# qope/SIPP

Measured on AMD Instinct MI355X. Metric: SIPP proof-gen wall-clock + pairings-aggregated/sec, n=128 (the 3 STARK sub-proofs, hardened G1/G2 AIRs; outer plonky2 proof not included), higher is better.
Workload: dtype u64; 1 GPU; n=128 SIPP instance per GPU: G1ExpStark 127 IO (N=2^16, W+P+Q=1176), G2ExpStark 127 IO (N=2^16, 2314), Fq12ExpStark 14 IO (N=2^13, 7970); IO records on host -> 3 flat proofs on host, the 3 sub-proofs on 3 concurrent HIP streams; parallelism=1 independent SIPP instance(s), one per GPU, no collective

## Files before the change

### sipp_amd/csrc/api.hip

```cpp
#include <algorithm>
#include <string>

#include "ctx.hpp"
#include "host_poseidon.hpp"

int sipp_poseidon_init_constants(sipp_ctx* ctx);

extern "C" {

void sipp_default_config(sipp_stark_config* cfg) {
    if (!cfg) return;
    cfg->rate_bits = 1;
    cfg->cap_height = 4;
    cfg->pow_bits = 16;
    cfg->arity_bits = 4;
    cfg->final_poly_bits = 5;
    cfg->num_queries = 84;
    cfg->num_challenges = 2;
    cfg->pow_rule = SIPP_POW_DUPLEX;
    cfg->fs_rule = SIPP_FS_STATEMENT;
    cfg->lookup_rule = SIPP_LOOKUP_INDEPENDENT;
}

static hipError_t create_ctx_stream(int device, int level, hipStream_t* out) {
    int lo = 0, hi = 0;
    (void)hipDeviceGetStreamPriorityRange(&lo, &hi);
    static const int dedicated = [] { const char* e = getenv("SIPP_DEDICATED_QUEUES"); return e ? atoi(e) : 1; }();
    if (level <= 0 && dedicated) {
        hipDeviceProp_t prop;
        if (hipGetDeviceProperties(&prop, device) == hipSuccess && prop.multiProcessorCount > 0 && prop.multiProcessorCount <= 1024) {
            uint32_t mask[32];
            const uint32_t words = ((uint32_t)prop.multiProcessorCount + 31) / 32;
            for (uint32_t i = 0; i < words; i++) {
                const uint32_t left = (uint32_t)prop.multiProcessorCount - 32 * i;
                mask[i] = left >= 32 ? 0xffffffffu : (1u << left) - 1;
            }
            if (hipExtStreamCreateWithCUMask(out, words, mask) == hipSuccess) return hipSuccess;
            (void)hipGetLastError();
        }
    }
    return hipStreamCreateWithPriority(out, hipStreamNonBlocking, level > 0 ? hi : level < 0 ? lo : 0);
}

int sipp_ctx_create(sipp_ctx** out, int device, const sipp_stark_config* cfg, size_t workspace_bytes) {
    if (!out) return SIPP_E_BADARG;
    *out = nullptr;
    int ndev = 0;
    if (hipGetDeviceCount(&ndev) != hipSuccess || ndev <= 0 || device < 0 || device >= ndev) return SIPP_E_HIP;
    sipp_ctx* ctx = new sipp_ctx();
    ctx->device = device;
    if (cfg)
        ctx->cfg = *cfg;
    else
        sipp_default_config(&ctx->cfg);
    if (ctx->cfg.rate_bits < 1 || ctx->cfg.rate_bits > 3 || ctx->cfg.num_challenges != 2 || ctx->cfg.arity_bits < 1 ||
        ctx->cfg.arity_bits > 4 || ctx->cfg.cap_height > 8 || ctx->cfg.pow_bits > 32 || ctx->cfg.pow_rule > SIPP_POW_HASH ||
        ctx->cfg.fs_rule > SIPP_FS_UPSTREAM || ctx->cfg.lookup_rule > SIPP_LOOKUP_SHARED || ctx->cfg.num_queries == 0 || ctx->cfg.num_queries > 1024 || ctx->cfg.final_poly_bits > 12) {
        delete ctx;
        return SIPP_E_UNSUPPORTED;
    }
    auto bail = [&](int rc) {
        hipError_t last = hipGetLastError();
        fprintf(stderr, "sipp_ctx_create(device %d, workspace %zu bytes) failed with status %d (last HIP error: %s)\n", device,
                workspace_bytes, rc, hipGetErrorString(last));
        sipp_ctx_destroy(ctx);
        return rc;
    };
    if (hipSetDevice(device) != hipSuccess) return bail(SIPP_E_HIP);
    if (create_ctx_stream(device, 0, &ctx->stream) != hipSuccess) return bail(SIPP_E_HIP);
    if (workspace_bytes == 0) workspace_bytes = (size_t)24 << 30;
    ctx->arena_size = workspace_bytes;
    if (hipMalloc((void**)&ctx->arena, workspace_bytes) != hipSuccess) return bail(SIPP_E_NOMEM);
    if (hipEventCreate(&ctx->t0) != hipSuccess || hipEventCreate(&ctx->t1) != hipSuccess) return bail(SIPP_E_HIP);
    ctx->h_pinned_words = (size_t)1 << 23;
    if (hipHostMalloc((void**)&ctx->h_pinned, ctx->h_pinned_words * 8) != hipSuccess) return bail(SIPP_E_NOMEM);
    int rc = sipp_poseidon_init_constants(ctx);
    if (rc != SIPP_OK) return bail(rc);
    *out = ctx;
    return SIPP_OK;
}

void sipp_ctx_destroy(sipp_ctx* ctx) {
    if (!ctx) return;
    if (ctx->async.started) {
        {
            std::unique_lock<std::mutex> lk(ctx->async.mu);
            ctx->async.cv.wait(lk, [&] { return !ctx->async.has_job || ctx->async.done; });
            ctx->async.quit = true;
        }
        ctx->async.cv.notify_all();
        ctx->async.th.join();
    }
    (void)hipSetDevice(ctx->device);
    if (ctx->stream) (void)hipStreamSynchronize(ctx->stream);
    sipp_witness_graph_release(ctx);
    for (auto& kv : ctx->tables) (void)hipFree(kv.second);
    for (auto e : ctx->ev_pool) (void)hipEventDestroy(e);
    if (ctx->t0) (void)hipEventDestroy(ctx->t0);
    if (ctx->t1) (void)hipEventDestroy(ctx->t1);
    if (ctx->h_pinned) (void)hipHostFree(ctx->h_pinned);
    if (ctx->arena) (void)hipFree(ctx->arena);
    if (ctx->aux_stream) (void)hipStreamDestroy(ctx->aux_stream);
    if (ctx->aux2_stream) (void)hipStreamDestroy(ctx->aux2_stream);
    if (ctx->stream) (void)hipStreamDestroy(ctx->stream);
    delete ctx;
}

uint32_t sipp_abi_version(void) { return SIPP_ABI_VERSION; }

int sipp_ctx_create_checked(sipp_ctx** out, int device, const sipp_stark_config* cfg, size_t cfg_size, uint32_t abi_version,
                            size_t workspace_bytes) {
    if (out) *out = nullptr;
    if (abi_version != SIPP_ABI_VERSION || (cfg && cfg_size != sizeof(sipp_stark_config))) return SIPP_E_BADARG;
    return sipp_ctx_create(out, device, cfg, workspace_bytes);
}

int sipp_ctx_set_kernel_routes(sipp_ctx* ctx, uint32_t routes) {
    if (!ctx || (routes & ~(uint32_t)(SIPP_ROUTE_OPENINGS_UNGROUPED | SIPP_ROUTE_LDE_COLUMN_WIDE | SIPP_ROUTE_WITNESS_NO_GRAPH))) return SIPP_E_BADARG;
    std::unique_lock<std::mutex> lk(ctx->async.mu);
    if (ctx->async.has_job) {
        lk.unlock();
        return sipp_fail(ctx, SIPP_E_BADARG, "set_kernel_routes: a proof is in flight on this ctx");
    }
    ctx->kernel_routes = routes;
    return SIPP_OK;
}

int sipp_ctx_set_hardened(sipp_ctx* ctx, int on) {
    if (!ctx) return SIPP_E_BADARG;
    std::unique_lock<std::mutex> lk(ctx->async.mu);
    if (ctx->async.has_job) {
        lk.unlock();
        return sipp_fail(ctx, SIPP_E_BADARG, "set_hardened: a proof is in flight on this ctx");
    }
    ctx->hardened = on != 0;
    return SIPP_OK;
}

int sipp_ctx_set_stream_priority(sipp_ctx* ctx, int level) {
    if (!ctx) return SIPP_E_BADARG;
    {
        std::unique_lock<std::mutex> lk(ctx->async.mu);
        if (ctx->async.has_job) {
            lk.unlock();
            return sipp_fail(ctx, SIPP_E_BADARG, "set_stream_priority: a proof is in flight on this ctx");
        }
    }
    SIPP_CHECK_HIP(ctx, hipSetDevice(ctx->device));
    hipStream_t ns = nullptr;
    if (create_ctx_stream(ctx->device, level, &ns) != hipSuccess) return sipp_fail(ctx, SIPP_E_HIP, "set_stream_priority: no stream");
    if (ctx->stream) {
        (void)hipStreamSynchronize(ctx->stream);
        if (ctx->prof) {
            (void)sipp_profile_enable(ctx, 0);
            ctx->prof = true;
        }
        (void)hipStreamDestroy(ctx->stream);
    }
    ctx->stream = ns;
    return SIPP_OK;
}

const char* sipp_last_error(const sipp_ctx* ctx) { return ctx ? ctx->err : "null ctx"; }

int sipp_sync(sipp_ctx* ctx) {
    if (!ctx) return SIPP_E_BADARG;
    SIPP_CHECK_HIP(ctx, hipSetDevice(ctx->device));
    SIPP_CHECK_HIP(ctx, hipStreamSynchronize(ctx->stream));
    return SIPP_OK;
}

void* sipp_stream(sipp_ctx* ctx) { return ctx ? (void*)ctx->stream : nullptr; }

static void prof_drain(sipp_ctx* ctx) {
    if (ctx->pending.empty()) return;
    (void)hipSetDevice(ctx->device);
    (void)hipStreamSynchronize(ctx->stream);
    for (auto& p : ctx->pending) {
        float ms = 0.f;
        if (hipEventElapsedTime(&ms, ctx->ev_pool[std::get<1>(p)], ctx->ev_pool[std::get<2>(p)]) == hipSuccess) {
            auto& e = ctx->prof_acc[std::get<0>(p)];
            e.calls++;
// ... 176 lines not shown
```

### sipp_amd/csrc/ctx.hpp

```cpp
#pragma once
#include <stdlib.h>
#include <hip/hip_runtime.h>
#include <stdint.h>
#include <stdio.h>
#include <string.h>

#include <condition_variable>
#include <map>
#include <mutex>
#include <string>
#include <thread>
#include <tuple>
#include <vector>

#include "../../include/sipp_hip.h"
#include "gl.hpp"

struct sipp_gate {
    std::mutex mu;
    std::condition_variable cv;
    bool open = false;
    void release() {
        {
            std::lock_guard<std::mutex> lk(mu);
            open = true;
        }
        cv.notify_all();
    }
    void wait() {
        std::unique_lock<std::mutex> lk(mu);
        cv.wait(lk, [&] { return open; });
    }
};

struct sipp_prof_entry {
    int calls = 0;
    double ms = 0.0;
};

struct sipp_ctx {
    int device = 0;
    hipStream_t stream = nullptr;
    sipp_stark_config cfg{};
    char err[512] = {0};

    char* arena = nullptr;
    size_t arena_size = 0;
    size_t arena_off = 0;
    size_t arena_peak = 0;

    std::map<std::tuple<int, uint64_t, uint64_t>, uint64_t*> tables;

    bool prof = false;
    std::vector<hipEvent_t> ev_pool;
    size_t ev_used = 0;
    std::vector<std::tuple<std::string, size_t, size_t>> pending;
    std::map<std::string, sipp_prof_entry> prof_acc;
    hipEvent_t t0 = nullptr, t1 = nullptr;

    uint64_t* h_pinned = nullptr;
    size_t h_pinned_words = 0;

    sipp_gate* gate_wait = nullptr;
    sipp_gate* gate_release = nullptr;

    hipStream_t aux_stream = nullptr;
    hipStream_t aux2_stream = nullptr;
    struct Fold {
        bool active = false;
        size_t mark = 0;
        uint32_t* d_ios[2] = {nullptr, nullptr};
        void* rows[2] = {nullptr, nullptr};
        int* d_err = nullptr;
        uint32_t num_io[2] = {0, 0};
        size_t n_in[2] = {0, 0};
    } fold;

    bool outputs_only = false;
    bool hardened = false;
    uint32_t kernel_routes = 0;
    struct WitnessGraph {
        hipGraph_t graph = nullptr;
        hipGraphExec_t exec = nullptr;
        std::vector<uint64_t> key;
    } wgraph;

    struct Async {
        std::thread th;
        std::mutex mu;
        std::condition_variable cv;
        bool started = false, has_job = false, done = false, quit = false;
        int kind = 0;
        const uint32_t* ios = nullptr;
        size_t num_io = 0, cap = 0, len = 0;
        uint64_t* out = nullptr;
        int rc = 0;
    } async;
};

#define SIPP_CHECK_HIP(ctx, expr)                                                                   \
    do {                                                                                            \
        hipError_t e__ = (expr);                                                                    \
        if (e__ != hipSuccess) {                                                                    \
            snprintf((ctx)->err, sizeof((ctx)->err), "%s:%d: %s -> %s", __FILE__, __LINE__, #expr,  \
                     hipGetErrorString(e__));                                                       \
            return SIPP_E_HIP;                                                                      \
        }                                                                                           \
    } while (0)

#define SIPP_TRY(expr)              \
    do {                            \
        int rc__ = (expr);          \
        if (rc__ != SIPP_OK) return rc__; \
    } while (0)

static inline int sipp_fail(sipp_ctx* ctx, int code, const char* msg) {
    if (ctx) snprintf(ctx->err, sizeof(ctx->err), "%s", msg);
    return code;
}

struct ArenaMark {
    size_t off;
};
static inline ArenaMark arena_mark(sipp_ctx* ctx) { return ArenaMark{ctx->arena_off}; }
static inline void arena_release(sipp_ctx* ctx, ArenaMark m) { ctx->arena_off = m.off; }
static inline void* arena_alloc(sipp_ctx* ctx, size_t bytes) {
    size_t off = (ctx->arena_off + 255) & ~(size_t)255;
    if (off + bytes > ctx->arena_size) {
        snprintf(ctx->err, sizeof(ctx->err), "workspace arena exhausted: need %zu more bytes (size %zu, used %zu)",
                 bytes, ctx->arena_size, off);
        return nullptr;
    }
    ctx->arena_off = off + bytes;
    if (ctx->arena_off > ctx->arena_peak) ctx->arena_peak = ctx->arena_off;
    return ctx->arena + off;
}
struct ArenaScope {
    sipp_ctx* ctx;
    ArenaMark mark;
    explicit ArenaScope(sipp_ctx* c) : ctx(c), mark(arena_mark(c)) {}
    ~ArenaScope() { arena_release(ctx, mark); }
    ArenaScope(const ArenaScope&) = delete;
    ArenaScope& operator=(const ArenaScope&) = delete;
};
// ... 86 lines not shown
```

### sipp_amd/csrc/fri.hip

```cpp
#include <algorithm>

#include "prover.hpp"

static size_t tree_words(uint32_t log_leaves) { return ((size_t)8 << log_leaves); }

static int read_cap(sipp_ctx* ctx, const uint64_t* d_tree, uint32_t log_leaves, uint32_t cap_height, uint64_t* cap_host) {
    const uint32_t ch = std::min(cap_height, log_leaves);
    uint64_t off = 0;
    for (uint32_t l = 0; l < log_leaves - ch; l++) off += (uint64_t)1 << (log_leaves - l);
    SIPP_CHECK_HIP(ctx, hipMemcpyAsync(cap_host, d_tree + 4 * off, ((size_t)4 << ch) * 8, hipMemcpyDeviceToHost, ctx->stream));
    SIPP_CHECK_HIP(ctx, hipStreamSynchronize(ctx->stream));
    return SIPP_OK;
}

size_t sipp_fri_core_words(const FriParamsDev& p, uint32_t log_n, const uint32_t* leaf_words, int n_oracles) {
    const uint32_t log_m = log_n + p.rate_bits;
    const size_t cap = (size_t)4 << p.cap_height;
    uint32_t sum = 0;
    for (uint32_t ab : p.arity_bits) sum += ab;
    size_t w = p.arity_bits.size() * cap + 2 * ((size_t)1 << (log_n - sum)) + 1;
    size_t per_q = 0;
    for (int o = 0; o < n_oracles; o++) per_q += leaf_words[o] + (size_t)(log_m - p.cap_height) * 4;
    uint32_t lt = log_m;
    for (uint32_t ab : p.arity_bits) {
        lt -= ab;
        per_q += ((size_t)2 << ab) + (size_t)(lt > p.cap_height ? lt - p.cap_height : 0) * 4;
    }
    return w + p.num_queries * per_q;
}

int sipp_fri_prove_core(sipp_ctx* ctx, const FriOracleDev* ors, int n_oracles, uint32_t log_n, const FriParamsDev& p,
                        uint64_t* d_final, host::Challenger& ch, uint64_t* pf, size_t& pos, size_t cap_total, size_t* final_len,
                        const std::function<void(const char*)>& tick) {
    const uint32_t log_m = log_n + p.rate_bits, R = (uint32_t)p.arity_bits.size(), nq = p.num_queries;
    const size_t n = (size_t)1 << log_n, m = (size_t)1 << log_m;
    const size_t cap_words = (size_t)4 << p.cap_height;
    if (p.cap_height > 8 || n_oracles < 1 || n_oracles > 8) return sipp_fail(ctx, SIPP_E_UNSUPPORTED, "fri: unsupported shape");
    auto push = [&](const uint64_t* v, size_t cnt) -> int {
        if (pos + cnt > cap_total) return SIPP_E_BUFSZ;
        memcpy(pf + pos, v, cnt * 8);
        pos += cnt;
        return SIPP_OK;
    };
    uint64_t cap_host[4 << 8];
    std::vector<uint64_t*> r_vals(R), r_tree(R);
    std::vector<uint32_t> r_loglen(R);
    uint64_t* cur = d_final;
    size_t len_c = n;
    uint32_t log_len = log_m;
    uint64_t shift = gl::GEN;
    for (uint32_t r = 0; r < R; r++) {
        const uint32_t ab = p.arity_bits[r];
        const size_t len = (size_t)1 << log_len;
        if (log_len < ab + 0u || (len_c >> ab) == 0) return sipp_fail(ctx, SIPP_E_BADARG, "fri: reduction arities exceed the degree");
        r_loglen[r] = log_len;
        r_vals[r] = arena_alloc_t<uint64_t>(ctx, 2 * len);
        r_tree[r] = arena_alloc_t<uint64_t>(ctx, tree_words(log_len - ab));
        uint64_t* nxt = arena_alloc_t<uint64_t>(ctx, 2 * (len_c >> ab) + 2);
        if (!r_vals[r] || !r_tree[r] || !nxt) return SIPP_E_NOMEM;
        SIPP_TRY(sipp_ntt_dif(ctx, cur, len_c, log_len - p.rate_bits, r_vals[r], len, log_len, 2, false, NttDiag{shift, 0}));
        SIPP_TRY(sipp_k_fri_leaves(ctx, r_vals[r], len, ab, r_tree[r]));
        SIPP_TRY(sipp_k_merkle_levels(ctx, r_tree[r], log_len - ab, p.cap_height));
        SIPP_TRY(read_cap(ctx, r_tree[r], log_len - ab, p.cap_height, cap_host));
        const size_t cw = (size_t)4 << std::min(p.cap_height, log_len - ab);
        ch.observe_many(cap_host, cw);
        SIPP_TRY(push(cap_host, cw));
        const gl::E2 fb = ch.get_ext();
        SIPP_TRY(sipp_k_fri_fold(ctx, cur, len_c, ab, fb, nxt));
        cur = nxt;
        len_c >>= ab;
        log_len -= ab;
        shift = gl::pow(shift, (uint64_t)1 << ab);
    }
    (void)cap_words;
    if (final_len) *final_len = len_c;
    {
        std::vector<uint64_t> fpv(2 * len_c);
        SIPP_CHECK_HIP(ctx, hipMemcpyAsync(fpv.data(), cur, fpv.size() * 8, hipMemcpyDeviceToHost, ctx->stream));
        SIPP_CHECK_HIP(ctx, hipStreamSynchronize(ctx->stream));
        for (size_t i = 0; i < len_c; i++) {
            uint64_t e[2] = {fpv[i], fpv[len_c + i]};
            ch.observe_many(e, 2);
            SIPP_TRY(push(e, 2));
        }
    }
    if (tick) tick("fri commit phase");
    uint64_t pow_witness = 0;
    if (p.pow_rule == SIPP_POW_HASH) {
        uint64_t zero[12] = {0}, cur_h[4];
        for (int i = 0; i < 4; i++) cur_h[i] = ch.get();
        SIPP_TRY(sipp_k_pow_search(ctx, zero, cur_h, 4, 0, p.pow_bits, &pow_witness));
    } else {
        SIPP_TRY(sipp_k_pow_search(ctx, ch.state, ch.in_buf, ch.n_in, 7, p.pow_bits, &pow_witness));
        ch.observe(pow_witness);
        (void)ch.get();
    }
    SIPP_TRY(push(&pow_witness, 1));
    if (tick) tick("pow");
    std::vector<uint32_t> qidx(nq);
    for (uint32_t i = 0; i < nq; i++) qidx[i] = (uint32_t)(ch.get() % m);
    uint32_t* d_idx = arena_alloc_t<uint32_t>(ctx, nq);
    if (!d_idx) return SIPP_E_NOMEM;
    SIPP_CHECK_HIP(ctx, hipMemcpyAsync(d_idx, qidx.data(), nq * 4, hipMemcpyHostToDevice, ctx->stream));
    const uint32_t nsib0 = log_m - p.cap_height;
    size_t st_words = 0;
    std::vector<size_t> off_rows(n_oracles), off_sib(n_oracles), off_leaf(R), off_rsib(R);
    std::vector<uint32_t> rsib(R), rshift(R);
    for (int o = 0; o < n_oracles; o++) {
        off_rows[o] = st_words;
        st_words += (size_t)nq * ors[o].ncols;
        off_sib[o] = st_words;
        st_words += (size_t)nq * nsib0 * 4;
    }
    {
        uint32_t sh = 0;
        for (uint32_t r = 0; r < R; r++) {
            const uint32_t ab = p.arity_bits[r];
            sh += ab;
            rshift[r] = sh;
            const uint32_t lt = log_m - sh;
            rsib[r] = lt > p.cap_height ? lt - p.cap_height : 0;
            off_leaf[r] = st_words;
            st_words += (size_t)nq * ((size_t)2 << ab);
            off_rsib[r] = st_words;
            st_words += (size_t)nq * rsib[r] * 4;
        }
    }
    if (st_words > ctx->h_pinned_words) return sipp_fail(ctx, SIPP_E_NOMEM, "query staging exceeds the pinned buffer");
    uint64_t* d_st = arena_alloc_t<uint64_t>(ctx, st_words);
    if (!d_st) return SIPP_E_NOMEM;
    std::vector<QueryGatherTask> tasks;
    {
        for (int o = 0; o < n_oracles; o++) {
            tasks.push_back(QueryGatherTask{ors[o].lde, d_st + off_rows[o], (uint64_t)ors[o].stride, 0, ors[o].ncols, 0, 0});
            if (nsib0) tasks.push_back(QueryGatherTask{ors[o].tree, d_st + off_sib[o], 0, 1, log_m, nsib0, 0});
        }
        for (uint32_t r = 0; r < R; r++) {
            const uint32_t ab = p.arity_bits[r];
            tasks.push_back(QueryGatherTask{r_vals[r], d_st + off_leaf[r], (uint64_t)1 << r_loglen[r], 2, rshift[r], ab, 0});
            if (rsib[r]) tasks.push_back(QueryGatherTask{r_tree[r], d_st + off_rsib[r], 0, 1, r_loglen[r] - ab, rsib[r], rshift[r]});
        }
        QueryGatherTask* d_tasks = arena_alloc_t<QueryGatherTask>(ctx, tasks.size());
        if (!d_tasks) return SIPP_E_NOMEM;
        SIPP_CHECK_HIP(ctx, hipMemcpyAsync(d_tasks, tasks.data(), tasks.size() * sizeof(QueryGatherTask), hipMemcpyHostToDevice, ctx->stream));
        SIPP_TRY(sipp_k_gather_tasks(ctx, d_tasks, (uint32_t)tasks.size(), d_idx, nq));
    }
    uint64_t* hst = ctx->h_pinned;
    SIPP_CHECK_HIP(ctx, hipMemcpyAsync(hst, d_st, st_words * 8, hipMemcpyDeviceToHost, ctx->stream));
    SIPP_CHECK_HIP(ctx, hipStreamSynchronize(ctx->stream));
    for (uint32_t qi = 0; qi < nq; qi++) {
        for (int o = 0; o < n_oracles; o++) {
            SIPP_TRY(push(hst + off_rows[o] + (size_t)qi * ors[o].ncols, (size_t)ors[o].ncols));
            SIPP_TRY(push(hst + off_sib[o] + (size_t)qi * nsib0 * 4, (size_t)nsib0 * 4));
        }
        for (uint32_t r = 0; r < R; r++) {
            const size_t lw = (size_t)2 << p.arity_bits[r];
            SIPP_TRY(push(hst + off_leaf[r] + (size_t)qi * lw, lw));
            SIPP_TRY(push(hst + off_rsib[r] + (size_t)qi * rsib[r] * 4, (size_t)rsib[r] * 4));
        }
    }
    return SIPP_OK;
}


#define SIPP_FRI_MAGIC 0x5349505046524931ULL

static size_t batch_len(const sipp_fri_batch& b) {
    size_t k = 0;
    for (uint32_t r = 0; r < b.n_ranges; r++) k += b.ranges[r].col_end - b.ranges[r].col_begin;
    return k;
}

static int check_params(sipp_ctx* ctx, const sipp_fri_params* p, uint32_t log_n) {
    if (!p || p->rate_bits < 1 || p->rate_bits > 3 || p->cap_height > 8 || p->pow_bits > 32 || p->pow_rule > SIPP_POW_HASH ||
        p->num_queries == 0 || p->num_queries > 1024 || p->n_rounds > SIPP_FRI_MAX_ROUNDS)
        return sipp_fail(ctx, SIPP_E_UNSUPPORTED, "fri: parameters out of the supported range");
    uint32_t sum = 0;
    for (uint32_t r = 0; r < p->n_rounds; r++) {
        if (p->arity_bits[r] < 1 || p->arity_bits[r] > 4) return sipp_fail(ctx, SIPP_E_UNSUPPORTED, "fri: arity must be 2, 4, 8 or 16");
        sum += p->arity_bits[r];
        if (log_n + p->rate_bits < sum + p->cap_height)
            return sipp_fail(ctx, SIPP_E_BADARG, "fri: reduction arities leave a layer smaller than its cap");
        if (log_n + p->rate_bits - sum + p->arity_bits[r] < 4)
            return sipp_fail(ctx, SIPP_E_UNSUPPORTED, "fri: a committed layer of fewer than 16 values is not supported");
    }
    if (sum > log_n) return sipp_fail(ctx, SIPP_E_BADARG, "fri: the reduction arities exceed the degree bits");
    if (log_n < 10 || log_n > 24) return sipp_fail(ctx, SIPP_E_UNSUPPORTED, "fri: degree bits outside the supported range [10, 24]");
    return SIPP_OK;
}

extern "C" {

void sipp_fri_const_arity(sipp_fri_params* p, uint32_t arity_bits, uint32_t final_poly_bits, uint32_t degree_bits) {
    if (!p) return;
    p->n_rounds = 0;
    while (degree_bits > final_poly_bits && degree_bits + p->rate_bits - arity_bits >= p->cap_height && degree_bits >= arity_bits &&
           p->n_rounds < SIPP_FRI_MAX_ROUNDS) {
        p->arity_bits[p->n_rounds++] = arity_bits;
        degree_bits -= arity_bits;
    }
}

int sipp_commit_batch_ex(sipp_ctx* ctx, const uint64_t* d_in, int from_coeffs, uint64_t* d_coeffs, uint64_t* d_lde, uint64_t* d_tree,
                         size_t ncols, uint32_t log_n, uint32_t rate_bits, uint32_t cap_height, const uint64_t* d_salt,
                         uint32_t n_salt, uint64_t* cap_out) {
    if (!ctx || !d_in || !d_coeffs || !d_lde || !d_tree || !cap_out || ncols == 0) return SIPP_E_BADARG;
    if (rate_bits < 1 || rate_bits > 3 || cap_height > 8 || (n_salt != 0 && (n_salt != SIPP_SALT_SIZE || !d_salt)))
        return sipp_fail(ctx, SIPP_E_UNSUPPORTED, "commit_batch_ex: blowup 2 / 4 / 8, cap height <= 8, salt 0 or 4 columns");
    SIPP_CHECK_HIP(ctx, hipSetDevice(ctx->device));
    const uint32_t log_m = log_n + rate_bits;
    const size_t n = (size_t)1 << log_n, m = (size_t)1 << log_m;
    ArenaScope scope(ctx);
    int rc;
    if (from_coeffs) {
        if (d_in != d_coeffs) SIPP_CHECK_HIP(ctx, hipMemcpyAsync(d_coeffs, d_in, ncols * n * 8, hipMemcpyDeviceToDevice, ctx->stream));
        rc = sipp_lde_from_coeffs(ctx, d_coeffs, d_lde, ncols, log_n, rate_bits);
        if (rc == SIPP_E_UNSUPPORTED) rc = sipp_ntt_dif(ctx, d_coeffs, n, log_n, d_lde, m, log_m, ncols, false, NttDiag{gl::GEN, 0});
    } else {
        rc = d_in != d_coeffs ? sipp_lde_from_values(ctx, d_in, d_coeffs, d_lde, ncols, log_n, rate_bits) : SIPP_E_UNSUPPORTED;
        if (rc == SIPP_E_UNSUPPORTED) {
            const uint64_t* src = d_in;
            if (d_in == d_coeffs) {
                uint64_t* tmp = arena_alloc_t<uint64_t>(ctx, n * ncols);
                if (!tmp) return SIPP_E_NOMEM;
                SIPP_CHECK_HIP(ctx, hipMemcpyAsync(tmp, d_in, n * ncols * 8, hipMemcpyDeviceToDevice, ctx->stream));
                src = tmp;
            }
            rc = sipp_bitrev_cols(ctx, src, n, d_coeffs, n, log_n, ncols);
            if (rc == SIPP_OK) rc = sipp_ntt_dit(ctx, d_coeffs, n, log_n, ncols, true, NttDiag{});
// ... 12 lines not shown
                           uint32_t log_n, const sipp_fri_params* p) {
    if (!oracles || !batches || !p || n_oracles == 0 || n_oracles > 8 || n_batches == 0) return 0;
    FriParamsDev fp;
    fp.rate_bits = p->rate_bits; fp.cap_height = p->cap_height; fp.pow_bits = p->pow_bits; fp.num_queries = p->num_queries;
    fp.pow_rule = p->pow_rule;
    uint32_t sum = 0;
    for (uint32_t r = 0; r < p->n_rounds && r < SIPP_FRI_MAX_ROUNDS; r++) {
        fp.arity_bits.push_back(p->arity_bits[r]);
        sum += p->arity_bits[r];
    }
    if (sum > log_n) return 0;
    uint32_t lw[8];
    for (size_t o = 0; o < n_oracles; o++) lw[o] = oracles[o].n_polys + oracles[o].n_salt;
    size_t w = 8 + sipp_fri_core_words(fp, log_n, lw, (int)n_oracles);
    for (size_t b = 0; b < n_batches; b++) w += 2 * batch_len(batches[b]);
    return w;
}

int sipp_fri_prove_openings(sipp_ctx* ctx, const sipp_oracle* oracles, size_t n_oracles, const sipp_fri_batch* batches,
                            size_t n_batches, uint32_t log_n, const sipp_fri_params* p, sipp_challenger* chs, uint64_t* proof_out,
                            size_t proof_cap, size_t* proof_len) {
    if (!ctx || !oracles || !batches || !p || !chs || !proof_out || !proof_len || n_oracles == 0 || n_oracles > 8 || n_batches == 0)
        return SIPP_E_BADARG;
    SIPP_CHECK_HIP(ctx, hipSetDevice(ctx->device));
    SIPP_TRY(check_params(ctx, p, log_n));
    if (chs->n_in > 7 || chs->n_out > 8) return sipp_fail(ctx, SIPP_E_BADARG, "fri: malformed challenger state");
    const size_t total = sipp_fri_proof_size(oracles, n_oracles, batches, n_batches, log_n, p);
    if (total == 0) return SIPP_E_BADARG;
    if (proof_cap < total) return sipp_fail(ctx, SIPP_E_BUFSZ, "fri: proof buffer too small (see sipp_fri_proof_size)");
    for (size_t b = 0; b < n_batches; b++)
        for (uint32_t r = 0; r < batches[b].n_ranges; r++) {
            const sipp_poly_range& rg = batches[b].ranges[r];
            if (rg.oracle >= n_oracles || rg.col_begin > rg.col_end || rg.col_end > oracles[rg.oracle].n_polys)
                return sipp_fail(ctx, SIPP_E_BADARG, "fri: polynomial range outside its oracle");
        }
    const size_t n = (size_t)1 << log_n, m = n << p->rate_bits;
    FriParamsDev fp;
    fp.rate_bits = p->rate_bits; fp.cap_height = p->cap_height; fp.pow_bits = p->pow_bits; fp.num_queries = p->num_queries;
    fp.pow_rule = p->pow_rule;
    for (uint32_t r = 0; r < p->n_rounds; r++) fp.arity_bits.push_back(p->arity_bits[r]);
    host::Challenger ch;
    memcpy(ch.state, chs->state, sizeof ch.state);
    memcpy(ch.in_buf, chs->in_buf, sizeof ch.in_buf);
    memcpy(ch.out_buf, chs->out_buf, sizeof ch.out_buf);
    ch.n_in = (uint32_t)chs->n_in;
    ch.n_out = (uint32_t)chs->n_out;
    struct Release {
        sipp_ctx* c;
        ArenaMark mk;
        ~Release() {
            (void)hipStreamSynchronize(c->stream);
            arena_release(c, mk);
        }
    } release{ctx, arena_mark(ctx)};
    size_t pos = 0;
    uint64_t* pf = proof_out;
    {
        uint64_t hdr[8] = {SIPP_FRI_MAGIC, p->n_rounds, 0, p->num_queries, (uint64_t)n_oracles, (uint64_t)n_batches, total, log_n};
        memcpy(pf, hdr, sizeof hdr);
        pos = 8;
    }
    std::vector<uint64_t*> d_zp(n_batches), d_zip(n_batches);
    std::vector<gl::E2> points(n_batches);
    for (size_t b = 0; b < n_batches; b++) {
        points[b] = gl::E2{batches[b].point[0], batches[b].point[1]};
        if (gl::eq(gl::pow(points[b], (uint64_t)n), gl::e2(1))) return sipp_fail(ctx, SIPP_E_SUBGROUP, "fri: opening point in the subgroup");
        d_zp[b] = arena_alloc_t<uint64_t>(ctx, 2 * n);
        d_zip[b] = arena_alloc_t<uint64_t>(ctx, 2 * n);
        if (!d_zp[b] || !d_zip[b]) return SIPP_E_NOMEM;
        SIPP_TRY(sipp_k_pow_table(ctx, points[b], n, d_zp[b]));
        SIPP_TRY(sipp_k_pow_table(ctx, gl::inv(points[b]), n, d_zip[b]));
    }
    for (size_t b = 0; b < n_batches; b++) {
        const size_t k = batch_len(batches[b]);
        uint64_t* d_open = arena_alloc_t<uint64_t>(ctx, 4 * k + 4);
        if (!d_open) return SIPP_E_NOMEM;
        size_t at = 0;
        for (uint32_t r = 0; r < batches[b].n_ranges; r++) {
            const sipp_poly_range& rg = batches[b].ranges[r];
            const size_t cnt = rg.col_end - rg.col_begin;
            SIPP_TRY(sipp_k_openings(ctx, oracles[rg.oracle].d_coeffs + (size_t)rg.col_begin * n, cnt, n, d_zp[b], nullptr, d_open + 4 * at));
            at += cnt;
        }
        std::vector<uint64_t> hop(4 * k + 4);
        SIPP_CHECK_HIP(ctx, hipMemcpyAsync(hop.data(), d_open, (4 * k) * 8, hipMemcpyDeviceToHost, ctx->stream));
        SIPP_CHECK_HIP(ctx, hipStreamSynchronize(ctx->stream));
        for (size_t j = 0; j < k; j++) {
            memcpy(pf + pos, &hop[4 * j], 16);
            pos += 2;
            ch.observe_many(&hop[4 * j], 2);
        }
    }
    const gl::E2 alpha = ch.get_ext();
    uint64_t* d_acc = arena_alloc_t<uint64_t>(ctx, 2 * n);
    uint64_t* d_final = arena_alloc_t<uint64_t>(ctx, 2 * n);
    if (!d_acc || !d_final) return SIPP_E_NOMEM;
    for (size_t b = 0; b < n_batches; b++) {
        const size_t k = batch_len(batches[b]);
        std::vector<const uint64_t*> cols;
        cols.reserve(k);
        for (uint32_t r = 0; r < batches[b].n_ranges; r++) {
            const sipp_poly_range& rg = batches[b].ranges[r];
            for (uint32_t c = rg.col_begin; c < rg.col_end; c++) cols.push_back(oracles[rg.oracle].d_coeffs + (size_t)c * n);
        }
        std::vector<uint32_t> apow(6 * k + 6);
        gl::E2 ap = gl::e2(1);
        for (size_t c = 0; c < k; c++) {
            const uint64_t comp[2] = {ap.c0, ap.c1};
            for (int q = 0; q < 2; q++) {
                apow[6 * c + 3 * q] = (uint32_t)comp[q] & 0x3FFFFFu;
                apow[6 * c + 3 * q + 1] = (uint32_t)(comp[q] >> 22) & 0x3FFFFFu;
                apow[6 * c + 3 * q + 2] = (uint32_t)(comp[q] >> 44);
            }
            ap = gl::mul(ap, alpha);
        }
        const uint64_t** d_cols = reinterpret_cast<const uint64_t**>(arena_alloc(ctx, (k + 1) * sizeof(uint64_t*)));
        uint32_t* d_apow = arena_alloc_t<uint32_t>(ctx, apow.size());
        if (!d_cols || !d_apow) return SIPP_E_NOMEM;
        SIPP_CHECK_HIP(ctx, hipMemcpyAsync(d_cols, cols.data(), k * sizeof(uint64_t*), hipMemcpyHostToDevice, ctx->stream));
        SIPP_CHECK_HIP(ctx, hipMemcpyAsync(d_apow, apow.data(), apow.size() * 4, hipMemcpyHostToDevice, ctx->stream));
        SIPP_CHECK_HIP(ctx, hipStreamSynchronize(ctx->stream));
        SIPP_TRY(sipp_k_fri_batch_quotient(ctx, d_cols, (int)k, n, d_apow, d_zp[b], d_zip[b], ap, b == 0, d_acc));
    }
    SIPP_TRY(sipp_k_fri_mulx(ctx, d_acc, n, d_final));
    FriOracleDev ors[8];
    for (size_t o = 0; o < n_oracles; o++)
        ors[o] = FriOracleDev{oracles[o].d_lde, m, oracles[o].n_polys + oracles[o].n_salt, oracles[o].d_tree};
    size_t flen = 0;
    SIPP_TRY(sipp_fri_prove_core(ctx, ors, (int)n_oracles, log_n, fp, d_final, ch, pf, pos, total, &flen, nullptr));
    pf[2] = flen;
    if (pos != total) return sipp_fail(ctx, SIPP_E_BUFSZ, "internal: opening proof length mismatch");
    *proof_len = pos;
    memcpy(chs->state, ch.state, sizeof ch.state);
    memcpy(chs->in_buf, ch.in_buf, sizeof ch.in_buf);
    memcpy(chs->out_buf, ch.out_buf, sizeof ch.out_buf);
    chs->n_in = ch.n_in;
    chs->n_out = ch.n_out;
    return SIPP_OK;
}

}
```

### sipp_amd/csrc/poseidon.hip

```cpp
#include <type_traits>
#include "ctx.hpp"
#ifndef GLL_T
#define GLL_T 140
#endif
#include "poseidon.hpp"
#include "poseidon_pair.hpp"
#include "prover.hpp"

namespace {

#ifndef SIPP_LEAVES_WPE
#define SIPP_LEAVES_WPE 3
#endif
__global__ void __launch_bounds__(256) __attribute__((amdgpu_waves_per_eu(SIPP_LEAVES_WPE, SIPP_LEAVES_WPE)))
poseidon_leaves_kernel(const uint64_t* __restrict__ lde, size_t col_stride,
                                                             uint32_t ncols, uint64_t n_leaves,
                                                             uint64_t* __restrict__ digests) {
    const uint64_t j0 = (uint64_t)blockIdx.x * blockDim.x + threadIdx.x;
    const uint64_t j = j0 < n_leaves ? j0 : n_leaves - 1;
    uint64_t s[12];
#pragma unroll
    for (int i = 0; i < 12; i++) s[i] = 0;
    const uint64_t* p = lde + j;
    __shared__ uint64_t stash[11 * 256];
// ... 190 lines not shown
    const uint32_t words = 2u << ab;
    const uint64_t* c0 = vals + (k << ab);
    const uint64_t* c1 = vals + len + (k << ab);
    uint64_t s[12];
#pragma unroll
    for (int i = 0; i < 12; i++) s[i] = 0;
    if (words <= 4) {
        s[0] = c0[0];
        s[1] = c1[0];
        if (words == 4) {
            s[2] = c0[1];
            s[3] = c1[1];
        }
    } else {
#pragma unroll 1
        for (uint32_t chunk = 0; chunk < words / 8; chunk++) {
#pragma unroll
            for (int e = 0; e < 8; e++) s[e] = (e & 1) ? c1[4 * chunk + (e >> 1)] : c0[4 * chunk + (e >> 1)];
            poseidon::permute(s);
        }
    }
    uint64_t* d = digests + 4 * k;
    d[0] = s[0]; d[1] = s[1]; d[2] = s[2]; d[3] = s[3];
}

struct PowArgs {
    uint64_t state[12];
    uint64_t in_buf[8];
    uint32_t n_in, pow_bits, resp_word;
    uint64_t base;
    unsigned long long* result;
};
__global__ void __launch_bounds__(256) pow_kernel(PowArgs a) {
    const uint64_t w = a.base + (uint64_t)blockIdx.x * blockDim.x + threadIdx.x;
    uint64_t s[12];
#pragma unroll
    for (int i = 0; i < 12; i++) s[i] = a.state[i];
#pragma unroll
    for (int i = 0; i < 8; i++) {
        if ((uint32_t)i < a.n_in) s[i] = a.in_buf[i];
        if ((uint32_t)i == a.n_in) s[i] = w;
    }
    poseidon::permute(s);
    const uint64_t resp = a.resp_word == 7 ? s[7] : s[0];
    if ((resp >> (64 - a.pow_bits)) == 0) atomicMin(a.result, (unsigned long long)w);
}

constexpr uint64_t thin_threshold() { return 65536; }

}

int sipp_k_fri_leaves(sipp_ctx* ctx, const uint64_t* d_vals, size_t len, uint32_t arity_bits, uint64_t* d_digests) {
    uint64_t nl = len >> arity_bits;
    ProfScope ps(ctx, "fri_leaves");
    if (arity_bits != 4) {
        if (arity_bits < 1 || arity_bits > 4) return sipp_fail(ctx, SIPP_E_UNSUPPORTED, "fri_leaves: arity must be 2, 4, 8 or 16");
        hipLaunchKernelGGL(fri_leaves_any_kernel, dim3((unsigned)((nl + 63) / 64)), dim3(64), 0, ctx->stream, d_vals, (uint64_t)len,
                           arity_bits, d_digests);
    } else if (nl <= thin_threshold())
        hipLaunchKernelGGL(fri_leaves_pair_kernel, dim3((unsigned)((2 * nl + 255) / 256)), dim3(256), 0, ctx->stream, d_vals,
                           (uint64_t)len, d_digests);
    else
        hipLaunchKernelGGL(fri_leaves_kernel, dim3((unsigned)((nl + 63) / 64)), dim3(64), 0, ctx->stream, d_vals, (uint64_t)len,
                           d_digests);
    SIPP_CHECK_HIP(ctx, hipGetLastError());
    return SIPP_OK;
}

int sipp_k_pow_search(sipp_ctx* ctx, const uint64_t state[12], const uint64_t* in_buf, uint32_t n_in, uint32_t resp_word,
                      uint32_t pow_bits, uint64_t* witness) {
    if (pow_bits == 0) { *witness = 0; return SIPP_OK; }
    if (pow_bits > 32 || n_in > 7 || (resp_word != 0 && resp_word != 7))
        return sipp_fail(ctx, SIPP_E_UNSUPPORTED, "pow_search: unsupported parameters");
    ArenaMark mk = arena_mark(ctx);
    unsigned long long* d_res = arena_alloc_t<unsigned long long>(ctx, 1);
    if (!d_res) return SIPP_E_NOMEM;
    PowArgs a;
    memcpy(a.state, state, sizeof a.state);
    memset(a.in_buf, 0, sizeof a.in_buf);
    memcpy(a.in_buf, in_buf, n_in * sizeof(uint64_t));
    a.n_in = n_in; a.pow_bits = pow_bits; a.resp_word = resp_word; a.result = d_res;
    const uint32_t log_batch = pow_bits + 1 < 12 ? 12 : pow_bits + 1 > 28 ? 28 : pow_bits + 1;
    const uint64_t batch = (uint64_t)1 << log_batch;
    unsigned long long h_res = ~0ull;
    SIPP_CHECK_HIP(ctx, hipMemsetAsync(d_res, 0xff, sizeof(unsigned long long), ctx->stream));
    for (uint64_t base = 0; base < ((uint64_t)1 << 44); base += batch) {
        a.base = base;
        {
            ProfScope ps(ctx, "pow_grind");
            hipLaunchKernelGGL(pow_kernel, dim3((unsigned)(batch / 256)), dim3(256), 0, ctx->stream, a);
        }
        SIPP_CHECK_HIP(ctx, hipGetLastError());
        SIPP_CHECK_HIP(ctx, hipMemcpyAsync(&h_res, d_res, sizeof h_res, hipMemcpyDeviceToHost, ctx->stream));
        SIPP_CHECK_HIP(ctx, hipStreamSynchronize(ctx->stream));
        if (h_res != ~0ull) break;
    }
    arena_release(ctx, mk);
    if (h_res == ~0ull) return sipp_fail(ctx, SIPP_E_UNSUPPORTED, "pow_search: no witness found");
    *witness = (uint64_t)h_res;
    return SIPP_OK;
}

int sipp_poseidon_init_constants(sipp_ctx* ctx) {
    SIPP_CHECK_HIP(ctx, hipMemcpyToSymbol(HIP_SYMBOL(poseidon::c_rc), SIPP_POSEIDON_RC, sizeof(SIPP_POSEIDON_RC)));
    SIPP_CHECK_HIP(ctx, hipMemcpyToSymbol(HIP_SYMBOL(poseidon::c_fast_first), SIPP_POSEIDON_FAST_FIRST,
                                          sizeof(SIPP_POSEIDON_FAST_FIRST)));
    SIPP_CHECK_HIP(ctx, hipMemcpyToSymbol(HIP_SYMBOL(poseidon::c_fast_scalar), SIPP_POSEIDON_FAST_SCALAR,
                                          sizeof(SIPP_POSEIDON_FAST_SCALAR)));
    SIPP_CHECK_HIP(ctx, hipMemcpyToSymbol(HIP_SYMBOL(poseidon::c_fast_mi), SIPP_POSEIDON_FAST_MI,
                                          sizeof(SIPP_POSEIDON_FAST_MI)));
    SIPP_CHECK_HIP(ctx, hipMemcpyToSymbol(HIP_SYMBOL(poseidon::c_fast_vs), SIPP_POSEIDON_FAST_VS,
                                          sizeof(SIPP_POSEIDON_FAST_VS)));
    SIPP_CHECK_HIP(ctx, hipMemcpyToSymbol(HIP_SYMBOL(poseidon::c_fast_what), SIPP_POSEIDON_FAST_WHAT,
                                          sizeof(SIPP_POSEIDON_FAST_WHAT)));
    SIPP_CHECK_HIP(ctx, hipMemcpyToSymbol(HIP_SYMBOL(poseidon::c_blk3), SIPP_POSEIDON_BLK3, sizeof(SIPP_POSEIDON_BLK3)));
    SIPP_CHECK_HIP(ctx, hipMemcpyToSymbol(HIP_SYMBOL(poseidon::c_comb3), SIPP_POSEIDON_COMB3, sizeof(SIPP_POSEIDON_COMB3)));
    SIPP_CHECK_HIP(ctx, hipMemcpyToSymbol(HIP_SYMBOL(poseidon::c_comb_c), SIPP_POSEIDON_COMB_C, sizeof(SIPP_POSEIDON_COMB_C)));
    SIPP_CHECK_HIP(ctx, hipMemcpyToSymbol(HIP_SYMBOL(poseidon::d_dense_a), SIPP_POSEIDON_DENSE_A, sizeof(SIPP_POSEIDON_DENSE_A)));
    SIPP_CHECK_HIP(ctx, hipMemcpyToSymbol(HIP_SYMBOL(poseidon::c_dense_start), SIPP_POSEIDON_DENSE_START, sizeof(SIPP_POSEIDON_DENSE_START)));
    SIPP_CHECK_HIP(ctx, hipMemcpyToSymbol(HIP_SYMBOL(poseidon_pair::d_pair_a), SIPP_POSEIDON_PAIR_A, sizeof(SIPP_POSEIDON_PAIR_A)));
    SIPP_CHECK_HIP(ctx, hipMemcpyToSymbol(HIP_SYMBOL(poseidon_pair::d_pair_mds_a), SIPP_POSEIDON_PAIR_MDS_A, sizeof(SIPP_POSEIDON_PAIR_MDS_A)));
    SIPP_CHECK_HIP(ctx, hipMemcpyToSymbol(HIP_SYMBOL(poseidon_pair::d_pair_cc), SIPP_POSEIDON_PAIR_CC3, sizeof(SIPP_POSEIDON_PAIR_CC3)));
    SIPP_CHECK_HIP(ctx, hipMemcpyToSymbol(HIP_SYMBOL(poseidon_pair::d_pair_start), SIPP_POSEIDON_PAIR_START, sizeof(SIPP_POSEIDON_PAIR_START)));
    return SIPP_OK;
}

int sipp_k_poseidon_leaves(sipp_ctx* ctx, const uint64_t* d_lde, size_t col_stride, size_t ncols, uint32_t log_leaves,
                           uint64_t* d_digests) {
    if (ncols == 0 || ncols > 0xffffffffull) return sipp_fail(ctx, SIPP_E_BADARG, "poseidon_leaves: bad ncols");
    uint64_t n = (uint64_t)1 << log_leaves;
    const bool thin = ncols > 4 && n <= thin_threshold() && n >= 32;
    ProfScope ps(ctx, ncols <= 4 ? "poseidon_leaves_noop" : thin ? "poseidon_leaves_pair" : "poseidon_leaves");
    if (ncols <= 4) {
        hipLaunchKernelGGL(poseidon_leaves_copy_kernel, dim3((unsigned)((n + 255) / 256)), dim3(256), 0, ctx->stream, d_lde, col_stride,
                           (uint32_t)ncols, n, d_digests);
    } else if (thin) {
        unsigned grid = (unsigned)((2 * n + 255) / 256);
        hipLaunchKernelGGL(poseidon_leaves_pair_kernel, dim3(grid), dim3(256), 0, ctx->stream, d_lde, col_stride,
                           (uint32_t)ncols, n, d_digests);
    } else {
        const unsigned bs = n <= 65536 ? 64 : 256;
        unsigned grid = (unsigned)((n + bs - 1) / bs);
        hipLaunchKernelGGL(poseidon_leaves_kernel, dim3(grid), dim3(bs), 0, ctx->stream, d_lde, col_stride,
                           (uint32_t)ncols, n, d_digests);
    }
    SIPP_CHECK_HIP(ctx, hipGetLastError());
    return SIPP_OK;
}

int sipp_k_merkle_levels(sipp_ctx* ctx, uint64_t* d_tree, uint32_t log_leaves, uint32_t cap_height) {
    if (cap_height > log_leaves) cap_height = log_leaves;
    {
        uint32_t level = 0;
        const uint32_t top = log_leaves - cap_height;
        while (level < top) {
            const uint32_t log_nodes = log_leaves - level;
            uint32_t lw = log_nodes <= 10 ? log_nodes : log_nodes >= 18 ? 10 : 8;
            uint32_t nlev = lw < top - level ? lw : top - level;
            const uint64_t widest_parents = (uint64_t)1 << (log_nodes - 1);
            if (widest_parents > thin_threshold()) {
                lw = 11;
                nlev = 3 < top - level ? 3 : top - level;
            }
            const unsigned blocks = 1u << (log_nodes - lw);
            ProfScope ps(ctx, "merkle_subtree");
            if (widest_parents <= thin_threshold())
                hipLaunchKernelGGL(merkle_subtree_kernel<true>, dim3(blocks), dim3(256), 0, ctx->stream, d_tree, log_leaves, level, lw, nlev);
            else
                hipLaunchKernelGGL(merkle_subtree_kernel<false>, dim3(blocks), dim3(256), 0, ctx->stream, d_tree, log_leaves, level, lw, nlev);
            SIPP_CHECK_HIP(ctx, hipGetLastError());
            level += nlev;
        }
        return SIPP_OK;
    }
}

// ... 9 lines not shown
```

### sipp_amd/csrc/prover.hip

```cpp
#include <map>

#include "ctx.hpp"
#include "prover.hpp"

namespace {

using gl::E2;

template <bool REV>
__device__ __forceinline__ uint64_t block_scan_mul_256(uint64_t v, uint64_t* s) {
    const int t = REV ? 255 - (int)threadIdx.x : (int)threadIdx.x;
    s[t] = v;
    __syncthreads();
    for (int off = 1; off < 256; off <<= 1) {
        uint64_t o = t >= off ? s[t - off] : 1;
        __syncthreads();
        v = gl::mul(v, o);
        s[t] = v;
        __syncthreads();
    }
    return v;
}

__device__ __forceinline__ void block_scan4_mul_256(uint64_t (&v)[4], uint64_t (*s)[256]) {
// ... 299 lines not shown
            const uint64_t coef = gl::from_i64(*w++);
            uint64_t va[16], vb[16];
            w += qvec<16>(w, c, va);
            w += qvec<16>(w, c, vb);
#pragma unroll
            for (int ch = 0; ch < 2; ch++) {
                gl::Acc6 Ae, Ao, Be, Bo;
                Ae.zero(); Ao.zero(); Be.zero(); Bo.zero();
#pragma unroll
                for (int i = 0; i < 8; i++) {
                    const uint32_t* g3 = a.ginv3[ch][i];
                    Ae.mac((uint32_t)va[2 * i], (uint32_t)(va[2 * i] >> 32), g3);
                    Ao.mac((uint32_t)va[2 * i + 1], (uint32_t)(va[2 * i + 1] >> 32), g3);
                    Be.mac((uint32_t)vb[2 * i], (uint32_t)(vb[2 * i] >> 32), g3);
                    Bo.mac((uint32_t)vb[2 * i + 1], (uint32_t)(vb[2 * i + 1] >> 32), g3);
                }
                const uint64_t ae = Ae.reduce(), ao = Ao.reduce(), be = Be.reduce(), bo = Bo.reduce();
                const uint64_t cross = gl::add(gl::mul(ae, bo), gl::mul(ao, be));
                uint64_t t = gl::mad(gl::mul(ao, bo), a.gamma_inv[ch], gl::mul(ae, be));
                t = gl::mad(cross, 65536, t);
                psum[ch] = gl::mad(coef, t, psum[ch]);
            }
        }
        const int nl = slice == 0 ? (int)*w++ : 0;
        for (int p = 0; p < nl; p++) {
            const uint64_t coef = gl::from_i64(*w++);
            uint64_t va[16];
            w += qvec<16>(w, c, va);
#pragma unroll
            for (int ii = 0; ii < 16; ii++) e[ii] = gl::mad(coef, va[ii], e[ii]);
        }
        if (slice == 0) {
        uint64_t q[17];
        (void)qvec<17>(qdesc, c, q);
        const uint64_t s = c.local(sign_col);
        const uint64_t sgn = gl::sub(1, gl::add(s, s));
        uint64_t cprev = 0;
        const uint64_t coff = gl::from_i64(coffset);
        uint64_t d[32];
#pragma unroll
        for (int k = 0; k < 32; k++) {
            uint64_t al = 0, ah = 0;
#pragma unroll
            for (int ii = 0; ii < 17; ii++) {
                const int jj = k - ii;
                if (jj >= 0 && jj < 16) {
                    al += (uint64_t)(uint32_t)q[ii] * a.p_limbs[jj];
                    ah += (uint64_t)(uint32_t)(q[ii] >> 32) * a.p_limbs[jj];
                }
            }
            const uint64_t l = al + (ah << 32);
            const uint32_t h = (uint32_t)(ah >> 32) + (l < al ? 1u : 0u);
            const uint64_t qp = gl::reduce96(h, l);
            d[k] = gl::sub(e[k], gl::mul(sgn, qp));
        }
        const uint64_t wgt = (uint64_t)1 << (16 * grp);
#pragma unroll
        for (int mm = 0; mm < 32; mm++) {
            if (mm < 32 / grp) {
                uint64_t v;
                if (grp == 2) v = gl::mad(d[(2 * mm + 1) & 31], 65536, d[(2 * mm) & 31]);
                else v = d[mm];
                uint64_t ck = 0;
                if (mm < 32 / grp - 1) {
                    for (int l = 0; l < ncl; l++)
                        ck = gl::mad(c.local(cbase + mm * ncl + l), (uint64_t)1 << (lb * l), ck);
                    ck = gl::sub(ck, coff);
                }
                v = gl::sub(v, cprev);
                v = gl::mad(ck, wgt, v);
                c.emit(v);
                cprev = ck;
            }
        }
        c.emit(gl::mul(s, gl::sub(s, 1)));
        }
        c.acc0 = gl::mad(a.alpha16[0], psum[0], c.acc0);
        c.acc1 = gl::mad(a.alpha16[1], psum[1], c.acc1);
    }
    a.part[((size_t)g * 2 + 0) * m + j] = gl::mul(c.acc0, a.seg_pow[2 * g]);
    a.part[((size_t)g * 2 + 1) * m + j] = gl::mul(c.acc1, a.seg_pow[2 * g + 1]);
}

__global__ void alpha_pow3_kernel(uint64_t a0, uint64_t a1, int K, int nc, uint32_t* __restrict__ out) {
    const int t = blockIdx.x * blockDim.x + threadIdx.x;
    const int total = 2 * 3 + nc * 2 * 6;
    if (t >= total) return;
    int c, e;
    if (t < 6) {
        c = t / 3;
        e = K - 1 - t % 3;
    } else {
        const int k = (t - 6) / 12, r = (t - 6) % 12, slot = r % 6;
        c = r / 6;
        e = K - 1 - (3 + 2 * k) - (slot >> 1) * 2 * nc - (slot & 1);
    }
    uint32_t l[3];
    gl::limbs3(l, gl::pow(c ? a1 : a0, (uint64_t)e));
    for (int q = 0; q < 3; q++) out[3 * t + q] = l[q];
}

struct RestAcc {
    gl::Acc6 a[2];
    int terms;
    uint64_t folded[2];
    __device__ __forceinline__ void init() {
        a[0].zero();
        a[1].zero();
        terms = 0;
        folded[0] = folded[1] = 0;
    }
    __device__ __forceinline__ void mac(uint64_t v, const uint32_t* __restrict__ p0, const uint32_t* __restrict__ p1) {
        const uint32_t lo = (uint32_t)v, hi = (uint32_t)(v >> 32);
        a[0].mac(lo, hi, p0);
        a[1].mac(lo, hi, p1);
    }
    __device__ __forceinline__ void maybe_fold(int added) {
        terms += added;
        if (terms >= 960) {
            for (int c = 0; c < 2; c++) {
                folded[c] = gl::add(folded[c], gl::canon(a[c].reduce()));
                a[c].zero();
            }
            terms = 0;
        }
    }
    __device__ __forceinline__ uint64_t value(int c) const { return gl::add(folded[c], gl::canon(a[c].reduce())); }
};

struct RestPoint {
    uint64_t lf, zl, ll, zh_inv;
};
__device__ __forceinline__ RestPoint rest_point(const QuotArgs& a, uint32_t i) {
    const uint64_t x = gl::mul(gl::GEN, gl::pow(a.w_m, i));
    const uint64_t zh = a.zh[i & 1];
    RestPoint r;
    r.zl = gl::sub(x, a.g_inv);
    r.lf = gl::mul(gl::mul(zh, a.ninv), gl::inv(gl::sub(x, 1)));
    r.ll = gl::mul(gl::mul(gl::mul(zh, a.ninv), a.g_inv), gl::inv(r.zl));
    r.zh_inv = a.zh_inv[i & 1];
    return r;
}
__device__ __forceinline__ void rest_store(const QuotArgs& a, size_t m, size_t j, const RestPoint& pt, const uint64_t F[2], const uint64_t T[2],
                                           const uint64_t R[2]) {
    uint64_t acc[2] = {0, 0};
    for (int g = 0; g < a.n_seg; g++) {
        acc[0] = gl::add(acc[0], a.part[((size_t)g * 2 + 0) * m + j]);
        acc[1] = gl::add(acc[1], a.part[((size_t)g * 2 + 1) * m + j]);
    }
#pragma unroll
    for (int q = 0; q < 2; q++) {
        uint64_t v = gl::mul(acc[q], a.alphaK[q]);
        v = gl::add(v, R[q]);
        v = gl::mad(pt.lf, F[q], v);
        v = gl::mad(pt.zl, T[q], v);
        a.out[(size_t)q * m + j] = gl::mul(v, pt.zh_inv);
    }
}

template <bool SPLIT>
__global__ void __launch_bounds__(256) quotient_rest_kernel(QuotArgs a) {
    const size_t m = (size_t)1 << a.log_m;
    constexpr uint32_t RB = 3, RW = 256u >> RB;
    const uint32_t tid = threadIdx.x, run = tid / RW, blk = blockIdx.x, half = blk / (uint32_t)(m >> 9);
    const size_t j = (size_t)half * (m >> 1) + (size_t)run * (m >> (RB + 1)) + (size_t)(blk % (uint32_t)(m >> 9)) * RW + tid % RW;
    const uint32_t i = gl::bitrev((uint32_t)j, a.log_m);
    QCtx c;
    c.lde = a.lde;
    c.lde_stride = a.lde_stride;
    c.alpha0 = a.alpha[0];
// ... 192 lines not shown
    } else {
        col = a.coeffs[2] + (size_t)(b - a.ncols[0] - a.ncols[1]) * a.n;
        t1 = nullptr;
    }
    openings_column(col, a.n, a.t0, t1, a.n, a.out + (size_t)b * 4);
}

constexpr int OG = 4;
struct OpenGArgs {
    const uint64_t* coeffs[3];
    uint32_t ncols[3];
    size_t n, seg_len;
    const uint64_t *t0, *t1;
    uint64_t* partial;
};
__global__ void __launch_bounds__(256) openings_group_kernel(OpenGArgs a) {
    __shared__ uint64_t s[4][256];
    uint32_t g = blockIdx.x, orc = 0, col_base = 0;
    while (orc < 2 && g >= (a.ncols[orc] + OG - 1) / OG) {
        g -= (a.ncols[orc] + OG - 1) / OG;
        col_base += a.ncols[orc];
        orc++;
    }
    const uint32_t c0 = g * OG, cnt = min((uint32_t)OG, a.ncols[orc] - c0);
    const bool two = orc < 2;
    const size_t n = a.n, lo = (size_t)blockIdx.y * a.seg_len, hi = min(n, lo + a.seg_len);
    const uint64_t* col = a.coeffs[orc] + (size_t)c0 * n;
    gl::Acc160 acc[OG][4];
    constexpr int OB = 2;
    size_t k = lo + threadIdx.x;
    for (; k + (OB - 1) * 256 < hi; k += OB * 256) {
        uint64_t p0[OB], p1[OB], q0[OB], q1[OB], v[OB][OG];
#pragma unroll
        for (int b = 0; b < OB; b++) {
            const size_t kb = k + (size_t)b * 256;
            p0[b] = a.t0[kb];
            p1[b] = a.t0[n + kb];
            q0[b] = two ? a.t1[kb] : 0;
            q1[b] = two ? a.t1[n + kb] : 0;
#pragma unroll
            for (int c = 0; c < OG; c++) v[b][c] = (uint32_t)c < cnt ? col[(size_t)c * n + kb] : 0;
        }
#pragma unroll
        for (int b = 0; b < OB; b++)
#pragma unroll
            for (int c = 0; c < OG; c++) {
                if ((uint32_t)c >= cnt) break;
                acc[c][0].mac(v[b][c], p0[b]);
                acc[c][1].mac(v[b][c], p1[b]);
                if (two) {
                    acc[c][2].mac(v[b][c], q0[b]);
                    acc[c][3].mac(v[b][c], q1[b]);
                }
            }
    }
    for (; k < hi; k += 256) {
        const uint64_t p0 = a.t0[k], p1 = a.t0[n + k], q0 = two ? a.t1[k] : 0, q1 = two ? a.t1[n + k] : 0;
#pragma unroll
        for (int c = 0; c < OG; c++) {
            if ((uint32_t)c >= cnt) break;
            const uint64_t v = col[(size_t)c * n + k];
            acc[c][0].mac(v, p0);
            acc[c][1].mac(v, p1);
            if (two) {
                acc[c][2].mac(v, q0);
                acc[c][3].mac(v, q1);
            }
        }
    }
#pragma unroll
    for (int c = 0; c < OG; c++) {
        if ((uint32_t)c >= cnt) break;
#pragma unroll
        for (int q = 0; q < 4; q++) s[q][threadIdx.x] = gl::canon(acc[c][q].reduce());
        __syncthreads();
        for (int off = 128; off > 0; off >>= 1) {
            if ((int)threadIdx.x < off)
                for (int q = 0; q < 4; q++) s[q][threadIdx.x] = gl::add(s[q][threadIdx.x], s[q][threadIdx.x + off]);
            __syncthreads();
        }
        if (threadIdx.x < 4) a.partial[((size_t)(col_base + c0 + c) * gridDim.y + blockIdx.y) * 4 + threadIdx.x] = s[threadIdx.x][0];
        __syncthreads();
    }
}

struct CombArgs {
    const uint64_t* src[3];
    int cnt[3];
    size_t n;
    const uint32_t* apow3;
    int n1;
    int slices;
    uint64_t* partial;
};
__global__ void __launch_bounds__(256) fri_combine_kernel(CombArgs a) {
    const size_t k = (size_t)blockIdx.x * 256 + threadIdx.x;
    const int total = a.cnt[0] + a.cnt[1] + a.cnt[2];
    const int per = (total + a.slices - 1) / a.slices;
    const int c_lo = blockIdx.y * per, c_hi = min(total, c_lo + per);
    gl::Acc6 G0, G1, H0, H1;
    G0.zero(); G1.zero(); H0.zero(); H1.zero();
    const uint64_t *src0 = a.src[0], *src1 = a.src[1], *src2 = a.src[2];
    const int cnt0 = a.cnt[0], cnt01 = a.cnt[0] + a.cnt[1], n1 = a.n1;
    const size_t nn = a.n;
    const uint32_t* __restrict__ apow3 = a.apow3;
    auto col_of = [=](int c) -> const uint64_t* {
        return c < cnt0 ? src0 + (size_t)c * nn : c < cnt01 ? src1 + (size_t)(c - cnt0) * nn : src2 + (size_t)(c - cnt01) * nn;
    };
#define SIPP_COMB_TERM(cc, vv)                                             \
    do {                                                                   \
        const uint64_t v_ = (vv);                                          \
        const uint32_t lo_ = (uint32_t)v_, hi_ = (uint32_t)(v_ >> 32);     \
        const uint32_t* __restrict__ w_ = apow3 + 6 * (cc);                \
        if ((cc) < n1) {                                 \
            G0.mac(lo_, hi_, w_);                                          \
            G1.mac(lo_, hi_, w_ + 3);                                      \
        } else {                                                           \
            H0.mac(lo_, hi_, w_);                                          \
            H1.mac(lo_, hi_, w_ + 3);                                      \
        }                                                                  \
    } while (0)
    constexpr int CB = 8;
    int c = c_lo;
    for (; c + CB <= c_hi; c += CB) {
        uint64_t v[CB];
#pragma unroll
        for (int b = 0; b < CB; b++) v[b] = col_of(c + b)[k];
#pragma unroll
        for (int b = 0; b < CB; b++) SIPP_COMB_TERM(c + b, v[b]);
    }
    for (; c < c_hi; c++) SIPP_COMB_TERM(c, col_of(c)[k]);
#undef SIPP_COMB_TERM
    const uint64_t g0 = gl::canon(G0.reduce()), g1 = gl::canon(G1.reduce());
    uint64_t* p = a.partial + (size_t)blockIdx.y * 4 * a.n;
    p[k] = gl::add(g0, gl::canon(H0.reduce()));
    p[a.n + k] = gl::add(g1, gl::canon(H1.reduce()));
    p[2 * a.n + k] = g0;
    p[3 * a.n + k] = g1;
}

struct GCombArgs {
    const uint64_t* const* cols;
    int total;
    size_t n;
    const uint32_t* apow3;
    int slices;
    uint64_t* partial;
};
__global__ void __launch_bounds__(256) fri_gcombine_kernel(GCombArgs a) {
    const size_t k = (size_t)blockIdx.x * 256 + threadIdx.x;
    const int per = (a.total + a.slices - 1) / a.slices;
    const int c_lo = blockIdx.y * per, c_hi = min(a.total, c_lo + per);
    gl::Acc6 G0, G1;
    G0.zero(); G1.zero();
    for (int c = c_lo; c < c_hi; c++) {
        const uint64_t v = a.cols[c][k];
        const uint32_t lo = (uint32_t)v, hi = (uint32_t)(v >> 32);
        const uint32_t* __restrict__ w = a.apow3 + 6 * c;
        G0.mac(lo, hi, w);
        G1.mac(lo, hi, w + 3);
    }
    uint64_t* p = a.partial + (size_t)blockIdx.y * 4 * a.n;
    p[k] = gl::canon(G0.reduce());
    p[a.n + k] = gl::canon(G1.reduce());
}

// ... 167 lines not shown
            const uint32_t l = e >> 2, w = e & 3;
            size_t off = 0;
            for (uint32_t k = 0; k < l; k++) off += (size_t)1 << (t.b - k);
            const size_t node = ((x >> t.d) >> l) ^ 1;
            t.out[((size_t)q * t.c + l) * 4 + w] = t.src[(off + node) * 4 + w];
        }
    } else {
        const size_t leaf = x >> t.b;
        for (uint32_t e = threadIdx.x; e < (2u << t.c); e += blockDim.x)
            t.out[((size_t)q << (t.c + 1)) + e] = t.src[(size_t)(e & 1) * t.a + (leaf << t.c) + (e >> 1)];
    }
}

}

int sipp_k_gather_tasks(sipp_ctx* ctx, const QueryGatherTask* d_tasks, uint32_t n_tasks, const uint32_t* d_idx, uint32_t nq) {
    if (!n_tasks || !nq) return SIPP_OK;
    ProfScope ps(ctx, "query_gather");
    hipLaunchKernelGGL(gather_tasks_kernel, dim3(nq, n_tasks), dim3(256), 0, ctx->stream, d_tasks, d_idx);
    SIPP_CHECK_HIP(ctx, hipGetLastError());
    return SIPP_OK;
}

int sipp_k_z_columns(sipp_ctx* ctx, const air_spec_t* a, const uint64_t* d_trace, uint32_t log_n, const uint64_t beta[2],
                     const uint64_t gamma[2], uint64_t* d_zv) {
    const size_t n = (size_t)1 << log_n;
    const int P = 2 * a->n_checked;
    const int zr = (n >= 16384) ? 8 : 4;
    const size_t zblock = (size_t)256 * zr;
    const unsigned nblk = (unsigned)(n / zblock);
    if (n % zblock) return sipp_fail(ctx, SIPP_E_BADARG, "z_columns: n must be a multiple of 1024");
    ArenaScope scope(ctx);
    uint64_t* totals = arena_alloc_t<uint64_t>(ctx, (size_t)2 * P * nblk);
    if (!totals) return SIPP_E_NOMEM;
    {
        ProfScope ps(ctx, "z_phase_a");
        if (zr == 8)
            hipLaunchKernelGGL(z_phase_a<8>, dim3(nblk, P / 2), dim3(256), 0, ctx->stream, d_trace, n, a->n_main, a->n_checked,
                               a->checked_base, gamma[0], gamma[1], beta[0], beta[1], d_zv, totals);
        else
            hipLaunchKernelGGL(z_phase_a<4>, dim3(nblk, P / 2), dim3(256), 0, ctx->stream, d_trace, n, a->n_main, a->n_checked,
                               a->checked_base, gamma[0], gamma[1], beta[0], beta[1], d_zv, totals);
    }
    {
        ProfScope ps(ctx, "z_phase_bc");
        hipLaunchKernelGGL(z_phase_b, dim3(P), dim3(256), 0, ctx->stream, totals, (int)nblk);
        if (zr == 8)
            hipLaunchKernelGGL(z_phase_c<8>, dim3(nblk, P), dim3(256), 0, ctx->stream, d_zv, n, totals);
        else
            hipLaunchKernelGGL(z_phase_c<4>, dim3(nblk, P), dim3(256), 0, ctx->stream, d_zv, n, totals);
    }
    SIPP_CHECK_HIP(ctx, hipGetLastError());
    return SIPP_OK;
}

static void host_ntt(uint64_t* a, uint32_t log_n, bool inverse) {
    const size_t n = (size_t)1 << log_n;
    for (size_t i = 0; i < n; i++) {
        const size_t j = gl::bitrev((uint32_t)i, log_n);
        if (i < j) std::swap(a[i], a[j]);
    }
    uint64_t root = gl::root_of_unity(log_n);
    if (inverse) root = gl::inv(root);
    for (uint32_t s = 1; s <= log_n; s++) {
        const size_t mlen = (size_t)1 << s, h = mlen >> 1;
        uint64_t wm = root;
        for (uint32_t k = s; k < log_n; k++) wm = gl::sqr(wm);
        for (size_t k = 0; k < n; k += mlen) {
            uint64_t w = 1;
            for (size_t j = 0; j < h; j++) {
                const uint64_t t = gl::mul(w, a[k + j + h]), u = a[k + j];
                a[k + j] = gl::add(u, t);
                a[k + j + h] = gl::sub(u, t);
                w = gl::mul(w, wm);
            }
        }
    }
    if (inverse) {
        const uint64_t ninv = gl::inv((uint64_t)n);
        for (size_t i = 0; i < n; i++) a[i] = gl::mul(a[i], ninv);
    }
}

int sipp_k_quotient(sipp_ctx* ctx, const air_spec_t* a, uint32_t log_n, const uint64_t* d_lde, const uint64_t* d_zlde,
                    size_t lde_stride, const uint64_t* d_aux, const uint64_t alpha[2], const uint64_t beta[2],
                    const uint64_t gamma[2], uint64_t* d_out) {
    const uint32_t log_m = log_n + 1;
    const size_t n = (size_t)1 << log_n, m = (size_t)1 << log_m;
    QuotArgs q{};
    q.lde = d_lde; q.zlde = d_zlde; q.aux = d_aux; q.lde_stride = lde_stride;
    q.prog = sipp_air_prog_device(ctx, a);
    if (!q.prog) return SIPP_E_HIP;
    q.prog_len = a->prog_len;
    q.W = a->n_main + 2 * a->n_checked; q.nm = a->n_main; q.nc = a->n_checked; q.cbase = a->checked_base;
    q.tbits = a->table_bits; q.log_n = log_n; q.log_m = log_m;
    q.alpha[0] = alpha[0]; q.alpha[1] = alpha[1]; q.gamma[0] = gamma[0]; q.gamma[1] = gamma[1];
    q.beta[0] = beta[0]; q.beta[1] = beta[1];
    const uint64_t g = gl::root_of_unity(log_n), wm = gl::root_of_unity(log_m);
    for (int k = 0; k < AIR_N_PERIODIC; k++) {
        const uint64_t mk = (uint64_t)AIR_PERIODIC[k][0], r0 = (uint64_t)AIR_PERIODIC[k][1];
        uint64_t* t = sipp_table_get(ctx, 200 + k, log_n, 0);
        if (!t) {
            const uint64_t K = n / mk;
            std::vector<uint64_t> v(2 * mk);
            const uint64_t gs = gl::inv(gl::pow(g, r0)), scale = gl::mul(K % gl::P, gl::inv(n % gl::P));
            for (uint64_t i = 0; i < 2 * mk; i++) {
                uint64_t x = gl::mul(gl::GEN, gl::pow(wm, i));
                uint64_t y = gl::mul(x, gs);
                uint64_t num = gl::sub(gl::pow(y, n), 1), den = gl::sub(gl::pow(y, K), 1);
                v[i] = gl::mul(gl::mul(num, gl::inv(den)), scale);
            }
            SIPP_TRY(sipp_table_put(ctx, 200 + k, log_n, 0, v, &t));
        }
        q.per_tab[k] = t;
        q.per_mask[k] = (uint32_t)(2 * mk - 1);
    }
    q.vper_tab = nullptr;
    q.vper_mask = 0;
    if (a->n_vflag + a->n_vconst > 0) {
        const uint32_t lr = (uint32_t)a->log_rows;
        const size_t R = (size_t)1 << lr, R2 = 2 * R;
        const int nv = a->n_vflag + a->n_vconst;
        uint64_t* t = sipp_table_get(ctx, 104, log_n, (uint64_t)a->kind);
        if (!t) {
            std::vector<uint64_t> tab((size_t)nv * R2), col(R2);
            const uint64_t shift = gl::pow(gl::GEN, (uint64_t)1 << (log_n - lr));
            std::map<std::vector<int64_t>, int> seen;
            std::vector<int64_t> vals(R);
            for (int k = 0; k < nv; k++) {
                for (size_t r = 0; r < R; r++) vals[r] = air_vper_value(a, k, (int)r);
                auto it = seen.find(vals);
                if (it != seen.end()) {
                    memcpy(&tab[(size_t)k * R2], &tab[(size_t)it->second * R2], R2 * 8);
                    continue;
                }
                seen.emplace(vals, k);
                for (size_t r = 0; r < R; r++) col[r] = gl::from_i64(vals[r]);
                host_ntt(col.data(), lr, true);
                uint64_t f = 1;
                for (size_t j = 0; j < R; j++) {
                    col[j] = gl::mul(col[j], f);
                    f = gl::mul(f, shift);
                }
                for (size_t j = R; j < R2; j++) col[j] = 0;
                host_ntt(col.data(), lr + 1, false);
                memcpy(&tab[(size_t)k * R2], col.data(), R2 * 8);
            }
            SIPP_TRY(sipp_table_put(ctx, 104, log_n, (uint64_t)a->kind, tab, &t));
        }
        q.vper_tab = t;
        q.vper_mask = (uint32_t)(R2 - 1);
    }
    const uint64_t sN = gl::pow(gl::GEN, n);
    q.zh[0] = gl::sub(sN, 1);
    q.zh[1] = gl::sub(gl::neg(sN), 1);
    q.zh_inv[0] = gl::inv(q.zh[0]);
    q.zh_inv[1] = gl::inv(q.zh[1]);
    q.ninv = gl::inv(n % gl::P);
    q.g_inv = gl::inv(g);
    q.w_m = wm;
    for (int i = 0; i < 16; i++) q.p_limbs[i] = AIR_BN_P_LIMBS[i];
    q.out = d_out;
    for (int ch = 0; ch < 2; ch++) {
        if (alpha[ch] == 0) return sipp_fail(ctx, SIPP_E_UNSUPPORTED, "quotient: a zero constraint challenge");
        const uint64_t gi = gl::inv(alpha[ch]);
        q.gamma_inv[ch] = gi;
        q.alpha16[ch] = gl::pow(alpha[ch], 16);
        uint64_t x = 1;
        for (int i = 0; i < 8; i++) {
            q.ginv3[ch][i][0] = (uint32_t)x & 0x3FFFFFu;
            q.ginv3[ch][i][1] = (uint32_t)(x >> 22) & 0x3FFFFFu;
            q.ginv3[ch][i][2] = (uint32_t)(x >> 44);
            x = gl::mul(x, gi);
        }
    }
    int n_gadget_segs = 0;
    ArenaScope scope(ctx);
    {
        std::vector<uint32_t> off, cnt;
        std::vector<int> ncons;
        const int64_t* w = a->prog;
        const int64_t* end = a->prog + a->prog_len;
        while (w < end && w[0] == 1) {
            off.push_back((uint32_t)(w - a->prog));
            cnt.push_back(0);
            if (w[6] != 2) return sipp_fail(ctx, SIPP_E_UNSUPPORTED, "quotient: gadgets must pair their limbs (group 2)");
            ncons.push_back(32 / (int)w[6] + 1);
            w += 7;
            w += 2 + 5 * w[1];
            int64_t np = *w++;
            for (int64_t p = 0; p < np; p++) {
                w += 1;
                w += 2 + 5 * w[1];
                w += 2 + 5 * w[1];
            }
            int64_t nl = *w++;
            for (int64_t p = 0; p < nl; p++) {
                w += 1;
                w += 2 + 5 * w[1];
            }
            if (np > 64) {
                const uint32_t nsl = (uint32_t)std::min<int64_t>(SIPP_QUOTIENT_MAX_SLICES, (np + 39) / 40);
                cnt.back() = 0x80000000u | (nsl << 8);
                for (uint32_t k = 1; k < nsl; k++) {
                    off.push_back(off.back());
                    cnt.push_back(0x80000000u | (nsl << 8) | k);
                    ncons.push_back(0);
                }
            }
        }
        while (w < end) {
            off.push_back((uint32_t)(w - a->prog));
            uint32_t k = 0;
            while (w < end && k < 64) {
                int64_t nmono = w[1];
                w += 2;
                for (int64_t mo = 0; mo < nmono; mo++) w += 2 + 2 * w[1];
                k++;
            }
            cnt.push_back(k);
            ncons.push_back((int)k);
        }
        const int ns = (int)off.size();
        q.n_seg = ns;
        n_gadget_segs = 0;
        auto is_gadget = [](uint32_t c) { return c == 0 || (c >> 31) != 0; };
        while (n_gadget_segs < ns && is_gadget(cnt[n_gadget_segs])) n_gadget_segs++;
        for (int g = n_gadget_segs; g < ns; g++)
            if (is_gadget(cnt[g])) return sipp_fail(ctx, SIPP_E_UNSUPPORTED, "quotient: gadgets must precede the polynomial constraints");
        std::vector<uint64_t> host((size_t)ns * 2 + ns + 2 + 192, 0);
        int after = 0;
        for (int g = ns - 1; g >= 0; g--) {
            host[2 * g] = gl::pow(alpha[0], (uint64_t)after);
            host[2 * g + 1] = gl::pow(alpha[1], (uint64_t)after);
            after += ncons[g];
        }
        uint32_t* h32 = reinterpret_cast<uint32_t*>(&host[2 * ns]);
        memcpy(h32, off.data(), (size_t)ns * 4);
        memcpy(h32 + ns, cnt.data(), (size_t)ns * 4);
        const size_t ap_at = (size_t)ns * 2 + (((size_t)2 * ns + 1) >> 1);
        {
            uint32_t* ap = reinterpret_cast<uint32_t*>(&host[ap_at]);
            for (int ch = 0; ch < 2; ch++) {
                uint64_t x = 1;
                for (int e = 0; e < 64; e++) {
                    ap[(ch * 64 + e) * 3 + 0] = (uint32_t)x & 0x3FFFFFu;
                    ap[(ch * 64 + e) * 3 + 1] = (uint32_t)(x >> 22) & 0x3FFFFFu;
                    ap[(ch * 64 + e) * 3 + 2] = (uint32_t)(x >> 44);
                    x = gl::mul(x, alpha[ch]);
                }
            }
        }
        uint64_t* d_tab = arena_alloc_t<uint64_t>(ctx, host.size());
        q.part = arena_alloc_t<uint64_t>(ctx, (size_t)ns * 2 * m);
        if (!d_tab || !q.part) return SIPP_E_NOMEM;
        SIPP_CHECK_HIP(ctx, hipMemcpyAsync(d_tab, host.data(), host.size() * 8, hipMemcpyHostToDevice, ctx->stream));
        SIPP_CHECK_HIP(ctx, hipStreamSynchronize(ctx->stream));
        q.seg_pow = d_tab;
        q.seg_off = reinterpret_cast<const uint32_t*>(d_tab + 2 * ns);
        q.seg_cnt = q.seg_off + ns;
        q.apoly3 = reinterpret_cast<const uint32_t*>(d_tab + ap_at);
    }
    {
        q.K = 3 + 6 * a->n_checked;
        const int nw = 6 + 12 * a->n_checked;
        uint32_t* d_ap = arena_alloc_t<uint32_t>(ctx, (size_t)3 * nw);
        if (!d_ap) return SIPP_E_NOMEM;
        hipLaunchKernelGGL(alpha_pow3_kernel, dim3((unsigned)((nw + 255) / 256)), dim3(256), 0, ctx->stream, alpha[0], alpha[1],
                           q.K, a->n_checked, d_ap);
        q.apow3 = d_ap;
        q.alphaK[0] = gl::pow(alpha[0], (uint64_t)q.K);
        q.alphaK[1] = gl::pow(alpha[1], (uint64_t)q.K);
    }
    {
        ProfScope ps(ctx, "quotient_prog");
        if (n_gadget_segs)
            hipLaunchKernelGGL(quotient_prog_kernel<false>, dim3((unsigned)(m / 64), (unsigned)n_gadget_segs), dim3(64), 0, ctx->stream, q, 0);
        if (q.n_seg > n_gadget_segs)
            hipLaunchKernelGGL(quotient_prog_kernel<true>, dim3((unsigned)(m / 64), (unsigned)(q.n_seg - n_gadget_segs)), dim3(64), 0, ctx->stream,
                               q, n_gadget_segs);
    }
    {
        ProfScope ps(ctx, "quotient_rest");
        q.chunks = (int)sipp_quotient_rest_chunks(log_n, a->n_checked);
        if (q.chunks > 1) {
            q.rest_part = arena_alloc_t<uint64_t>(ctx, (size_t)q.chunks * 6 * m);
            if (!q.rest_part) return SIPP_E_NOMEM;
            hipLaunchKernelGGL(quotient_rest_kernel<true>, dim3((unsigned)(m / 256), (unsigned)q.chunks), dim3(256), 0, ctx->stream, q);
            hipLaunchKernelGGL(quotient_finish_kernel, dim3((unsigned)(m / 256)), dim3(256), 0, ctx->stream, q);
        } else {
            q.chunks = 1;
            hipLaunchKernelGGL(quotient_rest_kernel<false>, dim3((unsigned)(m / 256)), dim3(256), 0, ctx->stream, q);
        }
    }
    SIPP_CHECK_HIP(ctx, hipGetLastError());
    return SIPP_OK;
}

int sipp_k_pow_table(sipp_ctx* ctx, gl::E2 base, size_t n, uint64_t* d_tab) {
    ProfScope ps(ctx, "pow_table");
    hipLaunchKernelGGL(pow_table_kernel, dim3((unsigned)((n + 255) / 256)), dim3(256), 0, ctx->stream, base, n, d_tab);
    SIPP_CHECK_HIP(ctx, hipGetLastError());
    return SIPP_OK;
}

int sipp_k_pow_table4(sipp_ctx* ctx, const gl::E2 base[4], size_t n, uint64_t* const d_tab[4]) {
    ProfScope ps(ctx, "pow_table");
    Pow4Args a;
    for (int i = 0; i < 4; i++) {
        a.base[i] = base[i];
        a.tab[i] = d_tab[i];
    }
    a.n = n;
    hipLaunchKernelGGL(pow_table4_kernel, dim3((unsigned)((n + 255) / 256), 4), dim3(256), 0, ctx->stream, a);
    SIPP_CHECK_HIP(ctx, hipGetLastError());
    return SIPP_OK;
}

int sipp_k_openings(sipp_ctx* ctx, const uint64_t* d_coeffs, size_t ncols, size_t n, const uint64_t* d_t0,
                    const uint64_t* d_t1, uint64_t* d_out) {
    if (!ncols) return SIPP_OK;
    ProfScope ps(ctx, "openings");
    const size_t want = (2048 + ncols - 1) / ncols, segs = std::min<size_t>(std::min<size_t>(64, want), n / 1024);
    if (segs <= 1) {
        hipLaunchKernelGGL(openings_kernel, dim3((unsigned)ncols), dim3(256), 0, ctx->stream, d_coeffs, n, (uint32_t)ncols, d_t0, d_t1,
                           d_out);
    } else {
        ArenaScope scope(ctx);
        uint64_t* partial = arena_alloc_t<uint64_t>(ctx, ncols * segs * 4);
        if (!partial) return SIPP_E_NOMEM;
        const size_t seg_len = (n + segs - 1) / segs;
        hipLaunchKernelGGL(openings_seg_kernel, dim3((unsigned)ncols, (unsigned)segs), dim3(256), 0, ctx->stream, d_coeffs, n, seg_len,
                           d_t0, d_t1, partial);
        hipLaunchKernelGGL(openings_fold_kernel, dim3((unsigned)((4 * ncols + 255) / 256)), dim3(256), 0, ctx->stream, partial,
                           (uint32_t)ncols, (uint32_t)segs, d_out);
    }
    SIPP_CHECK_HIP(ctx, hipGetLastError());
    return SIPP_OK;
}

int sipp_k_openings3(sipp_ctx* ctx, const uint64_t* const d_coeffs[3], const uint32_t ncols[3], size_t n, const uint64_t* d_t0,
                     const uint64_t* d_t1, uint64_t* d_out) {
    const unsigned total = ncols[0] + ncols[1] + ncols[2];
    if (!total) return SIPP_OK;
    ProfScope ps(ctx, "openings");
    Open3Args a;
    for (int i = 0; i < 3; i++) {
        a.coeffs[i] = d_coeffs[i];
        a.ncols[i] = ncols[i];
    }
    a.n = n; a.t0 = d_t0; a.t1 = d_t1; a.out = d_out;
    const bool grouped = !(ctx->kernel_routes & SIPP_ROUTE_OPENINGS_UNGROUPED);
    if (!grouped || n < 1024) {
        hipLaunchKernelGGL(openings3_kernel, dim3(total), dim3(256), 0, ctx->stream, a);
        SIPP_CHECK_HIP(ctx, hipGetLastError());
        return SIPP_OK;
    }
    OpenGArgs g;
    unsigned groups = 0;
    for (int i = 0; i < 3; i++) {
        g.coeffs[i] = d_coeffs[i];
        g.ncols[i] = ncols[i];
        groups += (ncols[i] + OG - 1) / OG;
    }
    const size_t segs = std::max<size_t>(1, std::min<size_t>(std::min<size_t>(SIPP_OPENINGS_MAX_SEGS, (4096 + groups - 1) / groups), n / 1024));
    ArenaScope scope(ctx);
    g.partial = arena_alloc_t<uint64_t>(ctx, (size_t)total * segs * 4);
    if (!g.partial) return SIPP_E_NOMEM;
    g.n = n; g.seg_len = (n + segs - 1) / segs; g.t0 = d_t0; g.t1 = d_t1;
    hipLaunchKernelGGL(openings_group_kernel, dim3(groups, (unsigned)segs), dim3(256), 0, ctx->stream, g);
    hipLaunchKernelGGL(openings_fold_kernel, dim3((4 * total + 255) / 256), dim3(256), 0, ctx->stream, g.partial, (uint32_t)total,
                       (uint32_t)segs, d_out);
    SIPP_CHECK_HIP(ctx, hipGetLastError());
    return SIPP_OK;
}

int sipp_k_fri_final(sipp_ctx* ctx, const uint64_t* const src[3], const int cnt[3], size_t n, const uint32_t* d_apow3,
                     int n1, gl::E2 shift1, const uint64_t* d_zp[2], const uint64_t* d_zip[2], uint64_t* d_final) {
    ArenaScope scope(ctx);
    const int total_cols = cnt[0] + cnt[1] + cnt[2];
    int slices = 8;
    while (slices < 64 && ((n / 256) * (size_t)slices < 2048 || (total_cols + slices - 1) / slices > 1024)) slices *= 2;
    uint64_t* partial = arena_alloc_t<uint64_t>(ctx, (size_t)slices * 4 * n);
    uint64_t* q = arena_alloc_t<uint64_t>(ctx, 4 * n);
    if (!partial || !q) return SIPP_E_NOMEM;
    CombArgs c{};
    for (int i = 0; i < 3; i++) { c.src[i] = src[i]; c.cnt[i] = cnt[i]; }
    c.n = n; c.apow3 = d_apow3; c.n1 = n1; c.slices = slices; c.partial = partial;
    if ((cnt[0] + cnt[1] + cnt[2] + slices - 1) / slices > 1024) return sipp_fail(ctx, SIPP_E_UNSUPPORTED, "fri_combine: more than 1024 columns per slice");
    {
        ProfScope ps(ctx, "fri_combine");
        hipLaunchKernelGGL(fri_combine_kernel, dim3((unsigned)(n / 256), slices), dim3(256), 0, ctx->stream, c);
    }
    DivArgs d{};
    d.partial = partial; d.slices = slices; d.n = n;
    d.zp[0] = d_zp[0]; d.zp[1] = d_zp[1]; d.zip[0] = d_zip[0]; d.zip[1] = d_zip[1];
    d.qout = q;
    const unsigned ntiles = (unsigned)(n / 1024);
    uint64_t* scan = arena_alloc_t<uint64_t>(ctx, 4 * n);
    uint64_t* totals = arena_alloc_t<uint64_t>(ctx, (size_t)4 * ntiles);
    if (!scan || !totals) return SIPP_E_NOMEM;
    if (n % 1024) return sipp_fail(ctx, SIPP_E_BADARG, "fri_divide: n must be a multiple of 1024");
    {
        ProfScope ps(ctx, "fri_divide");
        hipLaunchKernelGGL(fri_divide_tiles, dim3(ntiles, 2), dim3(1024), 0, ctx->stream, d, scan, totals);
        hipLaunchKernelGGL(fri_divide_carry, dim3(2), dim3(256), 0, ctx->stream, totals, (int)ntiles);
        hipLaunchKernelGGL(fri_divide_finish, dim3(ntiles, 2), dim3(1024), 0, ctx->stream, d, scan, totals);
        hipLaunchKernelGGL(fri_final_kernel, dim3((unsigned)((n + 255) / 256)), dim3(256), 0, ctx->stream, q, n, shift1, d_final);
    }
    SIPP_CHECK_HIP(ctx, hipGetLastError());
    return SIPP_OK;
}

int sipp_k_fri_batch_quotient(sipp_ctx* ctx, const uint64_t* const* d_cols, int total, size_t n, const uint32_t* d_apow3,
                              const uint64_t* d_zp, const uint64_t* d_zip, gl::E2 shift, bool first, uint64_t* d_acc) {
    ArenaScope scope(ctx);
    int slices = 1;
    while (slices < 64 && ((n / 256) * (size_t)slices < 1024 || (total + slices - 1) / slices > 1024)) slices *= 2;
    if ((total + slices - 1) / slices > 1024) return sipp_fail(ctx, SIPP_E_UNSUPPORTED, "fri: more than 65536 polynomials in one batch");
    if (n % 1024) return sipp_fail(ctx, SIPP_E_BADARG, "fri: degree must be a multiple of 1024");
    uint64_t* partial = arena_alloc_t<uint64_t>(ctx, (size_t)slices * 4 * n);
    uint64_t* q = arena_alloc_t<uint64_t>(ctx, 4 * n);
    uint64_t* scan = arena_alloc_t<uint64_t>(ctx, 4 * n);
    const unsigned ntiles = (unsigned)(n / 1024);
    uint64_t* totals = arena_alloc_t<uint64_t>(ctx, (size_t)4 * ntiles);
    if (!partial || !q || !scan || !totals) return SIPP_E_NOMEM;
    GCombArgs c{};
    c.cols = d_cols; c.total = total; c.n = n; c.apow3 = d_apow3; c.slices = slices; c.partial = partial;
    DivArgs d{};
    d.partial = partial; d.slices = slices; d.n = n;
    d.zp[0] = d_zp; d.zp[1] = d_zp; d.zip[0] = d_zip; d.zip[1] = d_zip;
    d.qout = q;
    {
        ProfScope ps(ctx, "fri_combine");
        hipLaunchKernelGGL(fri_gcombine_kernel, dim3((unsigned)(n / 256), slices), dim3(256), 0, ctx->stream, c);
    }
    {
        ProfScope ps(ctx, "fri_divide");
        hipLaunchKernelGGL(fri_divide_tiles, dim3(ntiles, 1), dim3(1024), 0, ctx->stream, d, scan, totals);
        hipLaunchKernelGGL(fri_divide_carry, dim3(1), dim3(256), 0, ctx->stream, totals, (int)ntiles);
        hipLaunchKernelGGL(fri_divide_finish, dim3(ntiles, 1), dim3(1024), 0, ctx->stream, d, scan, totals);
        hipLaunchKernelGGL(fri_accum_kernel, dim3((unsigned)((n + 255) / 256)), dim3(256), 0, ctx->stream, d_acc, q, n, shift, first ? 1 : 0);
    }
    SIPP_CHECK_HIP(ctx, hipGetLastError());
    return SIPP_OK;
}
int sipp_k_fri_mulx(sipp_ctx* ctx, const uint64_t* d_acc, size_t n, uint64_t* d_final) {
    hipLaunchKernelGGL(fri_mulx_kernel, dim3((unsigned)((n + 255) / 256)), dim3(256), 0, ctx->stream, d_acc, n, d_final);
    SIPP_CHECK_HIP(ctx, hipGetLastError());
    return SIPP_OK;
}

int sipp_k_fri_fold(sipp_ctx* ctx, const uint64_t* d_in, size_t len_in, uint32_t arity_bits, gl::E2 beta, uint64_t* d_out) {
    size_t len_out = len_in >> arity_bits;
    ProfScope ps(ctx, "fri_fold");
// ... 33 lines not shown
```

### sipp_amd/csrc/prover.hpp

```cpp
#pragma once
#include <functional>

#include "ctx.hpp"
#include "host_challenger.hpp"
#include "host_poseidon.hpp"
#include "poseidon_constants.h"

inline uint32_t sipp_quotient_rest_chunks(uint32_t log_n, int n_checked) {
    if (log_n + 1 > 15) return 1;
    const int c = n_checked / 32 < 16 ? n_checked / 32 : 16;
    return c > 1 ? (uint32_t)c : 1;
}
int sipp_k_z_columns(sipp_ctx* ctx, const air_spec_t* a, const uint64_t* d_trace, uint32_t log_n, const uint64_t beta[2],
                     const uint64_t gamma[2], uint64_t* d_zv);
int sipp_k_quotient(sipp_ctx* ctx, const air_spec_t* a, uint32_t log_n, const uint64_t* d_lde, const uint64_t* d_zlde,
                    size_t lde_stride, const uint64_t* d_aux, const uint64_t alpha[2], const uint64_t beta[2],
                    const uint64_t gamma[2], uint64_t* d_out);
int sipp_k_pow_table(sipp_ctx* ctx, gl::E2 base, size_t n, uint64_t* d_tab);
int sipp_k_pow_table4(sipp_ctx* ctx, const gl::E2 base[4], size_t n, uint64_t* const d_tab[4]);
int sipp_k_openings(sipp_ctx* ctx, const uint64_t* d_coeffs, size_t ncols, size_t n, const uint64_t* d_t0,
                    const uint64_t* d_t1, uint64_t* d_out);
constexpr size_t SIPP_OPENINGS_MAX_SEGS = 32;
constexpr int SIPP_QUOTIENT_MAX_SLICES = 8;
int sipp_k_openings3(sipp_ctx* ctx, const uint64_t* const d_coeffs[3], const uint32_t ncols[3], size_t n, const uint64_t* d_t0,
                     const uint64_t* d_t1, uint64_t* d_out);
int sipp_k_fri_final(sipp_ctx* ctx, const uint64_t* const src[3], const int cnt[3], size_t n, const uint32_t* d_apow3,
                     int n1, gl::E2 shift1, const uint64_t* d_zp[2], const uint64_t* d_zip[2], uint64_t* d_final);
int sipp_k_fri_batch_quotient(sipp_ctx* ctx, const uint64_t* const* d_cols, int total, size_t n, const uint32_t* d_apow3,
                              const uint64_t* d_zp, const uint64_t* d_zip, gl::E2 shift, bool first, uint64_t* d_acc);
int sipp_k_fri_mulx(sipp_ctx* ctx, const uint64_t* d_acc, size_t n, uint64_t* d_final);
int sipp_k_fri_fold(sipp_ctx* ctx, const uint64_t* d_in, size_t len_in, uint32_t arity_bits, gl::E2 beta, uint64_t* d_out);
struct QueryGatherTask {
    const uint64_t* src;
    uint64_t* out;
    uint64_t a;
    uint32_t type, b, c, d;
};
int sipp_k_gather_tasks(sipp_ctx* ctx, const QueryGatherTask* d_tasks, uint32_t n_tasks, const uint32_t* d_idx, uint32_t nq);
int sipp_k_gather_rows(sipp_ctx* ctx, const uint64_t* d_lde, size_t m, uint32_t ncols, const uint32_t* d_idx, uint32_t nq,
                       uint64_t* d_out);
int sipp_k_gather_siblings(sipp_ctx* ctx, const uint64_t* d_tree, uint32_t log_leaves, uint32_t nsib, uint32_t shift,
                           const uint32_t* d_idx, uint32_t nq, uint64_t* d_out);
int sipp_k_gather_fri_leaf(sipp_ctx* ctx, const uint64_t* d_vals, size_t len, uint32_t shift, uint32_t arity_bits,
                           const uint32_t* d_idx, uint32_t nq, uint64_t* d_out);
int sipp_k_fri_leaves(sipp_ctx* ctx, const uint64_t* d_vals, size_t len, uint32_t arity_bits, uint64_t* d_digests);
int sipp_k_pow_search(sipp_ctx* ctx, const uint64_t state[12], const uint64_t* in_buf, uint32_t n_in, uint32_t resp_word,
                      uint32_t pow_bits, uint64_t* witness);


struct FriOracleDev {
    const uint64_t* lde;
    size_t stride;
    uint32_t ncols;
    const uint64_t* tree;
};
struct FriParamsDev {
    uint32_t rate_bits = 1, cap_height = 4, pow_bits = 16, num_queries = 84, pow_rule = 0;
    std::vector<uint32_t> arity_bits;
};
size_t sipp_fri_core_words(const FriParamsDev& p, uint32_t log_n, const uint32_t* leaf_words, int n_oracles);
int sipp_fri_prove_core(sipp_ctx* ctx, const FriOracleDev* ors, int n_oracles, uint32_t log_n, const FriParamsDev& p,
                        uint64_t* d_final, host::Challenger& ch, uint64_t* pf, size_t& pos, size_t cap_total, size_t* final_len,
                        const std::function<void(const char*)>& tick);
```

### sipp_amd/csrc/stark.hip

```cpp
#include <atomic>
#include <thread>
#include <algorithm>
#include <chrono>

#include "prover.hpp"

static const int IO_WORDS[7] = {SIPP_G1_IO_WORDS, SIPP_G2_IO_WORDS, SIPP_FQ12_IO_WORDS, SIPP_MAP_G2_IO_WORDS, SIPP_G1_IO_WORDS, SIPP_G2_IO_WORDS,
                                SIPP_PAIRING_IO_WORDS};
static inline int base_kind(int kind) {
    return (kind == SIPP_G1_EXP_HARDENED || kind == SIPP_G2_EXP_HARDENED) ? kind - SIPP_G1_EXP_HARDENED : kind;
}
static inline int ctx_kind(const sipp_ctx* ctx, int kind) {
    return (ctx && ctx->hardened && (kind == SIPP_G1_EXP || kind == SIPP_G2_EXP)) ? kind + SIPP_G1_EXP_HARDENED : kind;
}
#define SIPP_MAGIC 0x5349505053544b31ULL

struct Shape {
    const air_spec_t* air;
    uint32_t log_n;
    uint32_t num_io;
    int W, P, Q;
};

static int shape_of(int kind, size_t num_io, Shape* s) {
    if (kind < 0 || kind > SIPP_PAIRING || num_io == 0 || num_io > ((size_t)1 << 17)) return SIPP_E_BADARG;
    const uint32_t log_rows = kind == SIPP_MAP_G2 ? 3 : kind == SIPP_PAIRING ? AIR_PAIRING_LOG_ROWS : 9;
    uint32_t nio = 2;
    while (nio < num_io || ((size_t)nio << log_rows) < 1024) nio <<= 1;
    uint32_t log_n = log_rows;
    while ((1u << (log_n - log_rows)) < nio) log_n++;
    s->air = sipp_air_get(kind, log_n);
    if (!s->air || (uint32_t)s->air->log_rows != log_rows) return SIPP_E_UNSUPPORTED;
    s->log_n = log_n;
    s->num_io = nio;
    s->W = s->air->n_main + 2 * s->air->n_checked;
    s->P = 2 * s->air->n_checked;
    s->Q = 4;
    return SIPP_OK;
}

static FriParamsDev fri_params_of(const sipp_stark_config& c, uint32_t degree_bits) {
    FriParamsDev p;
    p.rate_bits = c.rate_bits; p.cap_height = c.cap_height; p.pow_bits = c.pow_bits; p.num_queries = c.num_queries;
    p.pow_rule = c.pow_rule;
    while (degree_bits > c.final_poly_bits && degree_bits + c.rate_bits - c.arity_bits >= c.cap_height &&
           degree_bits >= c.arity_bits && p.arity_bits.size() < 32) {
        p.arity_bits.push_back(c.arity_bits);
        degree_bits -= c.arity_bits;
    }
    return p;
}

static size_t proof_words(const sipp_stark_config& cfg, const Shape& s) {
    const FriParamsDev fp = fri_params_of(cfg, s.log_n);
    const uint32_t log_m = s.log_n + cfg.rate_bits;
    const size_t cap = (size_t)4 << cfg.cap_height;
    size_t w = 16 + 3 * cap + 2 * (size_t)(2 * s.W + 2 * s.P + s.Q);
    const uint32_t leaf_words[3] = {(uint32_t)s.W, (uint32_t)s.P, (uint32_t)s.Q};
    w += sipp_fri_core_words(fp, s.log_n, leaf_words, 3);
    w += (size_t)s.num_io * s.air->pi_per_io;
    (void)log_m;
    return w;
}

static int upload_ios(sipp_ctx* ctx, int kind, const uint32_t* ios, size_t num_io, const Shape& s, uint32_t** d_ios,
                      std::vector<uint32_t>* host_copy) {
    const size_t ppi = IO_WORDS[kind];
    const size_t words = (size_t)s.num_io * ppi;
    if (words * 4 > ctx->h_pinned_words * 8) return sipp_fail(ctx, SIPP_E_NOMEM, "IO list larger than the pinned staging buffer");
    uint32_t* h = reinterpret_cast<uint32_t*>(ctx->h_pinned);
    for (size_t io = 0; io < s.num_io; io++)
        memcpy(h + io * ppi, ios + (io < num_io ? io : num_io - 1) * ppi, ppi * 4);
    if (host_copy) host_copy->assign(h, h + words);
    *d_ios = arena_alloc_t<uint32_t>(ctx, words);
    if (!*d_ios) return SIPP_E_NOMEM;
    SIPP_CHECK_HIP(ctx, hipMemcpyAsync(*d_ios, h, words * 4, hipMemcpyHostToDevice, ctx->stream));
    SIPP_CHECK_HIP(ctx, hipStreamSynchronize(ctx->stream));
    return SIPP_OK;
}

static size_t tree_words(uint32_t log_leaves) { return ((size_t)8 << log_leaves); }

static int read_cap(sipp_ctx* ctx, const uint64_t* d_tree, uint32_t log_leaves, uint64_t* cap_host) {
    const uint32_t ch = std::min(ctx->cfg.cap_height, log_leaves);
    uint64_t off = 0;
    for (uint32_t l = 0; l < log_leaves - ch; l++) off += (uint64_t)1 << (log_leaves - l);
    SIPP_CHECK_HIP(ctx, hipMemcpyAsync(cap_host, d_tree + 4 * off, ((size_t)4 << ch) * 8, hipMemcpyDeviceToHost, ctx->stream));
    SIPP_CHECK_HIP(ctx, hipStreamSynchronize(ctx->stream));
    return SIPP_OK;
}

static int commit_coeffs_launch(sipp_ctx* ctx, const uint64_t* d_coeffs, size_t ncols, uint32_t log_n, uint64_t* d_lde,
                                uint64_t* d_tree) {
    const uint32_t log_m = log_n + ctx->cfg.rate_bits;
    int rc = sipp_lde_from_coeffs(ctx, d_coeffs, d_lde, ncols, log_n, ctx->cfg.rate_bits);
    if (rc == SIPP_E_UNSUPPORTED)
        rc = sipp_ntt_dif(ctx, d_coeffs, (size_t)1 << log_n, log_n, d_lde, (size_t)1 << log_m, log_m, ncols, false,
                          NttDiag{gl::GEN, 0});
    SIPP_TRY(rc);
    SIPP_TRY(sipp_k_poseidon_leaves(ctx, d_lde, (size_t)1 << log_m, ncols, log_m, d_tree));
    return sipp_k_merkle_levels(ctx, d_tree, log_m, ctx->cfg.cap_height);
}
static int commit_coeffs(sipp_ctx* ctx, const uint64_t* d_coeffs, size_t ncols, uint32_t log_n, uint64_t* d_lde,
                         uint64_t* d_tree, uint64_t* cap_host) {
    SIPP_TRY(commit_coeffs_launch(ctx, d_coeffs, ncols, log_n, d_lde, d_tree));
    return read_cap(ctx, d_tree, log_n + ctx->cfg.rate_bits, cap_host);
}

static int commit_values_launch(sipp_ctx* ctx, const uint64_t* d_values, size_t ncols, uint32_t log_n, uint64_t* d_coeffs,
                                uint64_t* d_lde, uint64_t* d_tree) {
    const size_t n = (size_t)1 << log_n;
    const uint32_t log_m = log_n + ctx->cfg.rate_bits;
    const int rc = sipp_lde_from_values(ctx, d_values, d_coeffs, d_lde, ncols, log_n, ctx->cfg.rate_bits);
    if (rc == SIPP_OK) {
        SIPP_TRY(sipp_k_poseidon_leaves(ctx, d_lde, (size_t)1 << log_m, ncols, log_m, d_tree));
        return sipp_k_merkle_levels(ctx, d_tree, log_m, ctx->cfg.cap_height);
    }
    if (rc != SIPP_E_UNSUPPORTED) return rc;
    SIPP_TRY(sipp_bitrev_cols(ctx, d_values, n, d_coeffs, n, log_n, ncols));
    SIPP_TRY(sipp_ntt_dit(ctx, d_coeffs, n, log_n, ncols, true, NttDiag{}));
    return commit_coeffs_launch(ctx, d_coeffs, ncols, log_n, d_lde, d_tree);
}
static int commit_values(sipp_ctx* ctx, const uint64_t* d_values, size_t ncols, uint32_t log_n, uint64_t* d_coeffs,
                         uint64_t* d_lde, uint64_t* d_tree, uint64_t* cap_host) {
    SIPP_TRY(commit_values_launch(ctx, d_values, ncols, log_n, d_coeffs, d_lde, d_tree));
    return read_cap(ctx, d_tree, log_n + ctx->cfg.rate_bits, cap_host);
}

static void host_ifft(std::vector<uint64_t>& a, uint32_t log_n) {
    const size_t n = (size_t)1 << log_n;
    for (size_t i = 0; i < n; i++) {
        size_t j = gl::bitrev((uint32_t)i, log_n);
        if (i < j) std::swap(a[i], a[j]);
    }
    const uint64_t root = gl::inv(gl::root_of_unity(log_n));
    for (uint32_t s = 1; s <= log_n; s++) {
        const size_t mlen = (size_t)1 << s, h = mlen >> 1;
        uint64_t wm = root;
        for (uint32_t k = s; k < log_n; k++) wm = gl::sqr(wm);
        for (size_t k = 0; k < n; k += mlen) {
            uint64_t w = 1;
            for (size_t j = 0; j < h; j++) {
                uint64_t t = gl::mul(w, a[k + j + h]), u = a[k + j];
                a[k + j] = gl::add(u, t);
                a[k + j + h] = gl::sub(u, t);
                w = gl::mul(w, wm);
            }
        }
    }
    const uint64_t ninv = gl::inv((uint64_t)n);
    for (auto& v : a) v = gl::mul(v, ninv);
}

static void fq12_tower_limbs(const uint32_t* c96, int t, uint16_t limbs[16]) {
    static const uint64_t P[4] = {0x3c208c16d87cfd47ULL, 0x97816a916871ca8dULL, 0xb85045b68181585dULL, 0x30644e72e131a029ULL};
    typedef unsigned __int128 u128;
    const int i = t >> 1;
    uint64_t r[5] = {0, 0, 0, 0, 0};
    auto load = [&](int k, uint64_t out[4]) {
        for (int q = 0; q < 4; q++) out[q] = (uint64_t)c96[8 * k + 2 * q] | ((uint64_t)c96[8 * k + 2 * q + 1] << 32);
    };
    uint64_t hi[4];
    load(i + 6, hi);
    if (t & 1) {
        memcpy(r, hi, 32);
    } else {
        uint64_t lo[4];
        load(i, lo);
        u128 carry = 0;
        for (int q = 0; q < 4; q++) {
            carry += (u128)hi[q] * 9 + lo[q];
// ... 59 lines not shown
        }
    memcpy(root, d.data(), 32);
}

struct Oracle3 {
    uint64_t *coeffs, *lde, *tree;
    int ncols;
};

static int prove_impl(sipp_ctx* ctx, int kind, const uint32_t* ios, size_t num_io_in, uint64_t* proof_out, size_t proof_cap,
                      size_t* proof_len) {
    if (!ctx || !ios || !proof_out || !proof_len) return SIPP_E_BADARG;
    kind = ctx_kind(ctx, kind);
    struct GateGuard {
        sipp_ctx* c;
        ~GateGuard() {
            if (c->gate_release) c->gate_release->release();
            c->gate_release = nullptr;
        }
    } gate_guard{ctx};
    SIPP_CHECK_HIP(ctx, hipSetDevice(ctx->device));
    const sipp_stark_config& cfg = ctx->cfg;
    Shape s;
    SIPP_TRY(shape_of(kind, num_io_in, &s));
    const air_spec_t* a = s.air;
    const FriParamsDev fp = fri_params_of(cfg, s.log_n);
    const uint32_t log_n = s.log_n, log_m = log_n + cfg.rate_bits, R = (uint32_t)fp.arity_bits.size();
    if (R > 0 && log_m < (R - 1) * cfg.arity_bits + 4)
        return sipp_fail(ctx, SIPP_E_UNSUPPORTED, "stark: arity_bits / final_poly_bits fold the FRI layers below 16 values for this trace length");
    const uint32_t log_mq = log_n + 1;
    const size_t n = (size_t)1 << log_n, m = (size_t)1 << log_m, mq = (size_t)1 << log_mq;
    const size_t final_len = n >> (R * cfg.arity_bits);
    const int W = s.W, P = s.P, Q = s.Q;
    const uint32_t nq = cfg.num_queries;
    (void)nq;
    const size_t cap_words = (size_t)4 << cfg.cap_height;
    const size_t total_words = proof_words(cfg, s);
    if (proof_cap < total_words) return sipp_fail(ctx, SIPP_E_BUFSZ, "proof buffer too small (see sipp_proof_size)");
    if (n < ((size_t)1 << a->table_bits)) return sipp_fail(ctx, SIPP_E_UNSUPPORTED, "trace shorter than the range table");

    static const bool host_timing = getenv("SIPP_HOST_TIMING") != nullptr;
    auto t_prev = std::chrono::steady_clock::now();
    auto tick = [&](const char* what) {
        if (!host_timing) return;
        (void)hipStreamSynchronize(ctx->stream);
        auto now = std::chrono::steady_clock::now();
        fprintf(stderr, "[sipp kind %d] %-18s %8.3f ms\n", kind, what, std::chrono::duration<double, std::milli>(now - t_prev).count());
        t_prev = now;
    };
    ArenaMark mark = arena_mark(ctx);
    struct Release {
        sipp_ctx* c;
        ArenaMark m;
        ~Release() {
            (void)hipStreamSynchronize(c->stream);
            arena_release(c, m);
        }
    } release{ctx, mark};

    uint64_t* pf = proof_out;
    size_t pos = 0;
    auto push = [&](const uint64_t* v, size_t cnt) {
        memcpy(pf + pos, v, cnt * 8);
        pos += cnt;
    };
    {
        uint64_t hdr[16] = {SIPP_MAGIC, (uint64_t)kind, log_n, s.num_io, (uint64_t)W, (uint64_t)P, (uint64_t)Q, cfg.cap_height,
                            R, (uint64_t)final_len, nq, (uint64_t)a->pi_per_io, total_words, cfg.rate_bits, cfg.arity_bits,
                            (uint64_t)(cfg.fs_rule | (cfg.lookup_rule << 1))};
        push(hdr, 16);
    }

    std::vector<uint32_t> pis;
    uint32_t* d_ios = nullptr;
    SIPP_TRY(upload_ios(ctx, kind, ios, num_io_in, s, &d_ios, &pis));
    int* d_err = arena_alloc_t<int>(ctx, 1);
    uint64_t* d_trace = arena_alloc_t<uint64_t>(ctx, (size_t)W * n);
    Oracle3 T{arena_alloc_t<uint64_t>(ctx, (size_t)W * n), arena_alloc_t<uint64_t>(ctx, (size_t)W * m),
              arena_alloc_t<uint64_t>(ctx, tree_words(log_m)), W};
    Oracle3 Z{arena_alloc_t<uint64_t>(ctx, (size_t)P * n), arena_alloc_t<uint64_t>(ctx, (size_t)P * m),
              arena_alloc_t<uint64_t>(ctx, tree_words(log_m)), P};
    Oracle3 Qo{arena_alloc_t<uint64_t>(ctx, (size_t)2 * mq), arena_alloc_t<uint64_t>(ctx, (size_t)Q * m),
               arena_alloc_t<uint64_t>(ctx, tree_words(log_m)), Q};
    if (!d_err || !d_trace || !T.coeffs || !T.lde || !T.tree || !Z.coeffs || !Z.lde || !Z.tree || !Qo.coeffs || !Qo.lde ||
        !Qo.tree)
        return SIPP_E_NOMEM;
    if (!pis_canonical(kind, pis.data(), s.num_io))
        return sipp_fail(ctx, SIPP_E_WITNESS, "IO record holds a non-canonical field element (>= p)");
    SIPP_CHECK_HIP(ctx, hipMemsetAsync(d_err, 0, sizeof(int), ctx->stream));
    SIPP_TRY(sipp_trace_fill(ctx, a, d_ios, s.num_io, log_n, d_trace, d_err));
    {
        int h_err = 0;
        SIPP_CHECK_HIP(ctx, hipMemcpyAsync(&h_err, d_err, sizeof(int), hipMemcpyDeviceToHost, ctx->stream));
        SIPP_CHECK_HIP(ctx, hipStreamSynchronize(ctx->stream));
        if (h_err) return sipp_fail(ctx, h_err, "trace fill: IO record not provable (claimed output wrong, degenerate point or non-canonical limbs)");
    }

    tick("trace fill");
    if (ctx->gate_release) {
        ctx->gate_release->release();
        ctx->gate_release = nullptr;
    }
    if (ctx->gate_wait) {
        ctx->gate_wait->wait();
        ctx->gate_wait = nullptr;
    }
    uint64_t cap_host[4 << 8];

    SIPP_TRY(commit_values_launch(ctx, d_trace, (size_t)W, log_n, T.coeffs, T.lde, T.tree));
    host::Challenger ch;
    if (cfg.fs_rule == SIPP_FS_STATEMENT) {
        const uint64_t st[16] = {(uint64_t)kind, log_n, s.num_io, (uint64_t)W, (uint64_t)P, (uint64_t)Q, cfg.rate_bits,
                                 cfg.cap_height, cfg.pow_bits, cfg.arity_bits, cfg.final_poly_bits, cfg.num_queries,
                                 cfg.num_challenges, cfg.pow_rule, (uint64_t)a->pi_per_io, (uint64_t)cfg.lookup_rule};
        uint64_t root[4];
        ch.observe_many(st, 16);
        pi_root(pis.data(), s.num_io, a->pi_per_io, root);
        ch.observe_many(root, 4);
    }
    const int n_aux = a->n_aux;
    const uint32_t log_io = log_n - (uint32_t)a->log_rows;
    const size_t nio = s.num_io;
    std::vector<uint64_t> auxc((size_t)n_aux * nio), col(nio);
    {
        const uint64_t g = gl::root_of_unity(log_n);
        for (int ai = 0; ai < n_aux; ai++) {
            const int word = a->aux[4 * ai], part = a->aux[4 * ai + 1], shift = a->aux[4 * ai + 2], sub = a->aux[4 * ai + 3];
            for (size_t io = 0; io < nio; io++) {
                const uint32_t* rec = &pis[io * a->pi_per_io];
                if (part == 3) {
                    uint16_t limbs[16];
                    fq12_tower_limbs(rec + word, sub / 16, limbs);
                    col[io] = limbs[sub % 16];
                } else {
                    uint32_t w = rec[word];
                    col[io] = part == 0 ? (w & 0xffff) : part == 1 ? (w >> 16) : w;
                }
            }
            host_ifft(col, log_io);
            if (shift) {
                const uint64_t sft = gl::inv(gl::pow(g, (uint64_t)shift));
                uint64_t f = 1;
                for (size_t j = 0; j < nio; j++) {
                    col[j] = gl::mul(col[j], f);
                    f = gl::mul(f, sft);
                }
            }
            memcpy(&auxc[(size_t)ai * nio], col.data(), nio * 8);
        }
    }
    SIPP_TRY(read_cap(ctx, T.tree, log_m, cap_host));
    ch.observe_many(cap_host, cap_words);
    push(cap_host, cap_words);
    tick("trace commit");

    uint64_t beta[2], gamma[2];
    for (int i = 0; i < 2; i++) {
        beta[i] = ch.get();
        gamma[i] = ch.get();
        if (cfg.lookup_rule == SIPP_LOOKUP_SHARED) beta[i] = gamma[i];
    }
    {
        ArenaMark mz = arena_mark(ctx);
        uint64_t* d_zv = arena_alloc_t<uint64_t>(ctx, (size_t)P * n);
        if (!d_zv) return SIPP_E_NOMEM;
        SIPP_TRY(sipp_k_z_columns(ctx, a, d_trace, log_n, beta, gamma, d_zv));
        SIPP_TRY(commit_values(ctx, d_zv, (size_t)P, log_n, Z.coeffs, Z.lde, Z.tree, cap_host));
        arena_release(ctx, mz);
    }
    ch.observe_many(cap_host, cap_words);
    push(cap_host, cap_words);

    tick("Z + commit");
    uint64_t alpha[2];
    alpha[0] = ch.get();
    alpha[1] = ch.get();

    {
        ArenaMark mark_q = arena_mark(ctx);
        uint64_t* d_auxc = arena_alloc_t<uint64_t>(ctx, (size_t)n_aux * nio + 1);
        uint64_t* d_aux = arena_alloc_t<uint64_t>(ctx, (size_t)n_aux * mq + 1);
        if (!d_auxc || !d_aux) return SIPP_E_NOMEM;
        SIPP_CHECK_HIP(ctx, hipMemcpyAsync(d_auxc, auxc.data(), auxc.size() * 8, hipMemcpyHostToDevice, ctx->stream));
        SIPP_CHECK_HIP(ctx, hipStreamSynchronize(ctx->stream));
        if (n_aux) {
            int rc_aux = sipp_tree_coset_eval(ctx, d_auxc, d_aux, (size_t)n_aux, log_io, log_mq);
            if (rc_aux == SIPP_E_UNSUPPORTED)
                rc_aux = sipp_ntt_dif(ctx, d_auxc, nio, log_io, d_aux, mq, log_mq, (size_t)n_aux, false, NttDiag{gl::GEN, 0});
            SIPP_TRY(rc_aux);
        }
        SIPP_TRY(sipp_k_quotient(ctx, a, log_n, T.lde, Z.lde, m, d_aux, alpha, beta, gamma, Qo.coeffs));
        SIPP_TRY(sipp_ntt_dit(ctx, Qo.coeffs, mq, log_mq, 2, true, NttDiag{gl::inv(gl::GEN), 0}));
        SIPP_TRY(commit_coeffs(ctx, Qo.coeffs, (size_t)Q, log_n, Qo.lde, Qo.tree, cap_host));
        arena_release(ctx, mark_q);
    }
    ch.observe_many(cap_host, cap_words);
    push(cap_host, cap_words);

    tick("quotient + commit");
    const gl::E2 zeta = ch.get_ext();
    if (gl::eq(gl::pow(zeta, (uint64_t)n), gl::e2(1))) return sipp_fail(ctx, SIPP_E_SUBGROUP, "zeta in the trace subgroup");
    const gl::E2 gzeta = gl::scale(zeta, gl::root_of_unity(log_n));
    uint64_t* d_zp[2] = {arena_alloc_t<uint64_t>(ctx, 2 * n), arena_alloc_t<uint64_t>(ctx, 2 * n)};
    uint64_t* d_zip[2] = {arena_alloc_t<uint64_t>(ctx, 2 * n), arena_alloc_t<uint64_t>(ctx, 2 * n)};
    uint64_t* d_open = arena_alloc_t<uint64_t>(ctx, (size_t)(W + P + Q) * 4);
    if (!d_zp[0] || !d_zp[1] || !d_zip[0] || !d_zip[1] || !d_open) return SIPP_E_NOMEM;
    {
        const gl::E2 bases[4] = {zeta, gzeta, gl::inv(zeta), gl::inv(gzeta)};
        uint64_t* const tabs[4] = {d_zp[0], d_zp[1], d_zip[0], d_zip[1]};
        SIPP_TRY(sipp_k_pow_table4(ctx, bases, n, tabs));
    }
    {
        const uint64_t* const cf[3] = {T.coeffs, Z.coeffs, Qo.coeffs};
        const uint32_t nc3[3] = {(uint32_t)W, (uint32_t)P, (uint32_t)Q};
        SIPP_TRY(sipp_k_openings3(ctx, cf, nc3, n, d_zp[0], d_zp[1], d_open));
    }
    std::vector<uint64_t> hop((size_t)(W + P + Q) * 4);
    SIPP_CHECK_HIP(ctx, hipMemcpyAsync(hop.data(), d_open, hop.size() * 8, hipMemcpyDeviceToHost, ctx->stream));
    SIPP_CHECK_HIP(ctx, hipStreamSynchronize(ctx->stream));
    {
        for (int c = 0; c < W; c++) push(&hop[(size_t)c * 4], 2);
        for (int c = 0; c < W; c++) push(&hop[(size_t)c * 4 + 2], 2);
        for (int c = 0; c < P; c++) push(&hop[(size_t)(W + c) * 4], 2);
        for (int c = 0; c < P; c++) push(&hop[(size_t)(W + c) * 4 + 2], 2);
        for (int c = 0; c < Q; c++) push(&hop[(size_t)(W + P + c) * 4], 2);
        for (int c = 0; c < W; c++) ch.observe_many(&hop[(size_t)c * 4], 2);
        for (int c = 0; c < P; c++) ch.observe_many(&hop[(size_t)(W + c) * 4], 2);
        for (int c = 0; c < Q; c++) ch.observe_many(&hop[(size_t)(W + P + c) * 4], 2);
        for (int c = 0; c < W; c++) ch.observe_many(&hop[(size_t)c * 4 + 2], 2);
        for (int c = 0; c < P; c++) ch.observe_many(&hop[(size_t)(W + c) * 4 + 2], 2);
    }

    tick("openings+observe");
    const gl::E2 fa = ch.get_ext();
    uint64_t* d_final = arena_alloc_t<uint64_t>(ctx, 2 * n);
    {
        std::vector<uint32_t> apow((size_t)(W + P + Q) * 6);
        gl::E2 ap = gl::e2(1);
        for (int c = 0; c < W + P + Q; c++) {
            const uint64_t comp[2] = {ap.c0, ap.c1};
            for (int q = 0; q < 2; q++) {
                apow[6 * c + 3 * q] = (uint32_t)comp[q] & 0x3FFFFFu;
                apow[6 * c + 3 * q + 1] = (uint32_t)(comp[q] >> 22) & 0x3FFFFFu;
                apow[6 * c + 3 * q + 2] = (uint32_t)(comp[q] >> 44);
            }
            ap = gl::mul(ap, fa);
        }
        uint32_t* d_apow = arena_alloc_t<uint32_t>(ctx, apow.size());
        if (!d_final || !d_apow) return SIPP_E_NOMEM;
        SIPP_CHECK_HIP(ctx, hipMemcpyAsync(d_apow, apow.data(), apow.size() * 4, hipMemcpyHostToDevice, ctx->stream));
        SIPP_CHECK_HIP(ctx, hipStreamSynchronize(ctx->stream));
        const uint64_t* src[3] = {T.coeffs, Z.coeffs, Qo.coeffs};
        const int cnt[3] = {W, P, Q};
        const uint64_t* zp[2] = {d_zp[0], d_zp[1]};
        const uint64_t* zip[2] = {d_zip[0], d_zip[1]};
        SIPP_TRY(sipp_k_fri_final(ctx, src, cnt, n, d_apow, W + P, gl::pow(fa, (uint64_t)(W + P)), zp, zip, d_final));
    }
    {
        const FriOracleDev ors[3] = {{T.lde, m, (uint32_t)W, T.tree}, {Z.lde, m, (uint32_t)P, Z.tree}, {Qo.lde, m, (uint32_t)Q, Qo.tree}};
        size_t flen = 0;
        SIPP_TRY(sipp_fri_prove_core(ctx, ors, 3, log_n, fp, d_final, ch, pf, pos, total_words, &flen, tick));
        if (flen != final_len) return sipp_fail(ctx, SIPP_E_BUFSZ, "internal: final polynomial length mismatch");
    }
    for (size_t k = 0; k < pis.size(); k++) pf[pos++] = pis[k];
    tick("queries+assemble");
    if (pos != total_words) return sipp_fail(ctx, SIPP_E_BUFSZ, "internal: proof length mismatch");
    *proof_len = pos;
    return SIPP_OK;
}

extern "C" {

int sipp_stark_shape(const sipp_ctx* ctx, int kind, size_t num_io, uint32_t* log_rows, uint32_t* main_cols,
                     uint32_t* perm_cols, uint32_t* quotient_cols) {
    kind = ctx_kind(ctx, kind);
    Shape s;
    SIPP_TRY(shape_of(kind, num_io, &s));
    if (log_rows) *log_rows = s.log_n;
    if (main_cols) *main_cols = (uint32_t)s.W;
    if (perm_cols) *perm_cols = (uint32_t)s.P;
    if (quotient_cols) *quotient_cols = (uint32_t)s.Q;
    return SIPP_OK;
}

int sipp_io_shard(size_t num_io, uint32_t world, uint32_t rank, size_t* first, size_t* count) {
    if (!first || !count || world == 0 || rank >= world || num_io > SIZE_MAX / world) return SIPP_E_BADARG;
    const size_t lo = num_io * rank / world, hi = num_io * ((size_t)rank + 1) / world;
    *first = lo;
    *count = hi - lo;
    return SIPP_OK;
}

size_t sipp_workspace_bytes(int kind, size_t num_io) { return sipp_workspace_bytes_cfg(kind, num_io, nullptr); }

int sipp_device_memory(int device, size_t* free_bytes, size_t* total_bytes) {
    int ndev = 0;
    if (hipGetDeviceCount(&ndev) != hipSuccess || device < 0 || device >= ndev) return SIPP_E_HIP;
    int prev = 0;
    (void)hipGetDevice(&prev);
    size_t fr = 0, tot = 0;
    if (hipSetDevice(device) != hipSuccess || hipMemGetInfo(&fr, &tot) != hipSuccess) return SIPP_E_HIP;
    (void)hipSetDevice(prev);
    if (free_bytes) *free_bytes = fr;
    if (total_bytes) *total_bytes = tot;
    return SIPP_OK;
}

size_t sipp_workspace_bytes_cfg(int kind, size_t num_io, const sipp_stark_config* cfg) {
    Shape s;
    if (shape_of(kind, num_io, &s) != SIPP_OK) return 0;
    const uint32_t rate_bits = cfg ? cfg->rate_bits : 1;
    if (rate_bits < 1 || rate_bits > 3) return 0;
    const size_t n = (size_t)1 << s.log_n, m = n << rate_bits;
    const size_t W = (size_t)s.W, P = (size_t)s.P, Q = (size_t)s.Q, nc = (size_t)s.air->n_checked;
    size_t words = n * (2 * W + 3 * P)
                   + m * (W + P + Q + 2 + (size_t)s.air->n_aux)
                   + 3 * 8 * m
                   + 2 * m * (1 + (size_t)s.air->n_gadgets + (size_t)s.air->n_constraints / 64 + 2 +
                              (kind == SIPP_PAIRING ? SIPP_QUOTIENT_MAX_SLICES : 0))
                   + (sipp_quotient_rest_chunks(s.log_n, s.air->n_checked) > 1
                          ? (size_t)sipp_quotient_rest_chunks(s.log_n, s.air->n_checked) * 6 * 2 * n : 0)
                   + (W + P + Q) * SIPP_OPENINGS_MAX_SEGS * 4
                   + 80 * n;
    size_t bytes = 8 * words + nc * ((size_t)16 << s.air->table_bits)
                   + n * 400
                   + ((size_t)64 << 20);
    return bytes + bytes / 16;
}

size_t sipp_proof_size(const sipp_ctx* ctx, int kind, size_t num_io) {
    kind = ctx_kind(ctx, kind);
    Shape s;
    if (!ctx || shape_of(kind, num_io, &s) != SIPP_OK) return 0;
    return proof_words(ctx->cfg, s);
// ... 372 lines not shown
```

### sipp_amd/csrc/trace.hip

```cpp
#include <algorithm>

#include "air_tables.h"
#include "ctx.hpp"
#include "fq.hpp"

namespace {

using fq::Fq;
using fq::Fq2;

template <int EXT>
struct Fld;
template <>
struct Fld<1> {
    using T = Fq;
    static __device__ __forceinline__ T add(const T& a, const T& b) { return fq::add(a, b); }
    static __device__ __forceinline__ T sub(const T& a, const T& b) { return fq::sub(a, b); }
    static __device__ __forceinline__ T mul(const T& a, const T& b) { return fq::mul(a, b); }
    static __device__ __forceinline__ T sqr(const T& a) { return fq::sqr(a); }
    static __device__ __forceinline__ T inv(const T& a) { return fq::inv(a); }
    static __device__ __forceinline__ bool is_zero(const T& a) { return fq::is_zero(a); }
    static __device__ __forceinline__ T load(const uint32_t* w) {
        Fq r;
#pragma unroll
// ... 1102 lines not shown
            for (int q = 0; q < 8; q++) {
                const uint32_t i = hs + j + 64 * q;
                pi[i] = hv;
                pt[i] = (j + 64 * q) == 0 ? hv : f[q];
            }
        }
        for (; j < hc; j += 64) {
            const uint32_t i = hs + j, k = i - hd;
            pi[i] = hv;
            pt[i] = j == 0 ? hv : (k < nz ? zl[k] : T - 1);
        }
    }
}

}

const air_spec_t* sipp_air_get(int kind, uint32_t log_n) {
    const bool u16 = log_n >= 16;
    if (kind < 0 || kind > 6) return nullptr;
    const int hard = (kind == 4 || kind == 5) ? 1 : 0, base = hard ? kind - 4 : kind;
    for (size_t i = 0; i < sizeof(AIR_AIRS) / sizeof(AIR_AIRS[0]); i++)
        if (AIR_AIRS[i].kind == base && AIR_AIRS[i].hardened == hard && (AIR_AIRS[i].table_bits == 16) == u16) return &AIR_AIRS[i];
    return nullptr;
}

static int64_t* prog_on_device(sipp_ctx* ctx, const air_spec_t* a) {
    uint64_t* t = sipp_table_get(ctx, 100, (uint64_t)(a->kind + 8 * a->hardened), (uint64_t)a->table_bits);
    if (t) return (int64_t*)t;
    std::vector<uint64_t> v(a->prog_len);
    memcpy(v.data(), a->prog, (size_t)a->prog_len * 8);
    if (sipp_table_put(ctx, 100, (uint64_t)(a->kind + 8 * a->hardened), (uint64_t)a->table_bits, v, &t) != SIPP_OK) return nullptr;
    return (int64_t*)t;
}
const int64_t* sipp_air_prog_device(sipp_ctx* ctx, const air_spec_t* a) { return prog_on_device(ctx, a); }
const int8_t* sipp_air_vflag_device(sipp_ctx* ctx, const air_spec_t* a) {
    if (a->n_vflag == 0) return nullptr;
    uint64_t* t = sipp_table_get(ctx, 103, (uint64_t)a->kind, 0);
    if (!t) {
        const size_t bytes = (size_t)a->n_vflag << a->log_rows;
        std::vector<uint64_t> v((bytes + 7) / 8, 0);
        int8_t* f = reinterpret_cast<int8_t*>(v.data());
        for (int k = 0; k < a->n_vflag; k++)
            for (int r = 0; r < (1 << a->log_rows); r++) f[((size_t)k << a->log_rows) + (size_t)r] = (int8_t)air_vper_value(a, k, r);
        if (sipp_table_put(ctx, 103, (uint64_t)a->kind, 0, v, &t) != SIPP_OK) return nullptr;
    }
    return reinterpret_cast<const int8_t*>(t);
}

size_t sipp_curve_rows_bytes(int kind, uint32_t log_n) {
    return ((size_t)1 << log_n) * (kind == 0 ? sizeof(RowPts<1>) : sizeof(RowPts<2>));
}

size_t sipp_fold_rows_bytes(int kind, uint32_t num_io) {
    return (size_t)num_io * 512 * (kind == 0 ? sizeof(RowPts<1>) : sizeof(RowPts<2>));
}
int sipp_fold_chain_begin(sipp_ctx* ctx, int kind, const uint32_t* d_ios, uint32_t num_io, uint32_t ppi, void* rows, hipStream_t st) {
    if (kind == 0)
        hipLaunchKernelGGL((curve_dbl_par_kernel<1, 4>), dim3((num_io + 15) / 16), dim3(64), 0, st, d_ios, num_io, ppi,
                           reinterpret_cast<RowPts<1>*>(rows));
    else
        hipLaunchKernelGGL((curve_dbl_par_kernel<2, 8>), dim3((num_io + 7) / 8), dim3(64), 0, st, d_ios, num_io, ppi,
                           reinterpret_cast<RowPts<2>*>(rows));
    SIPP_CHECK_HIP(ctx, hipGetLastError());
    return SIPP_OK;
}
int sipp_fold_chain_finish(sipp_ctx* ctx, int kind, uint32_t* d_ios, uint32_t num_io, uint32_t ppi, void* rows, int* d_err,
                           hipStream_t st) {
    if (kind == 0) {
        hipLaunchKernelGGL(curve_scan_kernel<1>, dim3(num_io), dim3(256), 0, st, d_ios, num_io, ppi, reinterpret_cast<RowPts<1>*>(rows));
        hipLaunchKernelGGL(curve_outputs_kernel<1>, dim3((num_io + 63) / 64), dim3(64), 0, st, reinterpret_cast<RowPts<1>*>(rows), d_ios,
                           num_io, ppi, d_err);
    } else {
        hipLaunchKernelGGL(curve_scan_kernel<2>, dim3(num_io), dim3(256), 0, st, d_ios, num_io, ppi, reinterpret_cast<RowPts<2>*>(rows));
        hipLaunchKernelGGL(curve_outputs_kernel<2>, dim3((num_io + 63) / 64), dim3(64), 0, st, reinterpret_cast<RowPts<2>*>(rows), d_ios,
                           num_io, ppi, d_err);
    }
    SIPP_CHECK_HIP(ctx, hipGetLastError());
    return SIPP_OK;
}

static void gate_after_chain(sipp_ctx* ctx) {
    if (ctx->gate_wait) {
        ctx->gate_wait->wait();
        ctx->gate_wait = nullptr;
    }
}

int sipp_trace_fill(sipp_ctx* ctx, const air_spec_t* a, const uint32_t* d_ios, uint32_t num_io, uint32_t log_n,
                    uint64_t* d_trace, int* d_err) {
    const size_t n = (size_t)1 << log_n;
    const int cpl = a->cells_per_limb, nm = a->n_main, nc = a->n_checked;
    ArenaScope scope(ctx);
    int col_bit = 0, col_e = 0, exp_off = 0;
    const bool exp_air = a->kind != 3 && a->kind != 6;
    if (a->kind == 3) {
        if (ctx->outputs_only) {
            SIPP_TRY(sipp_mapg2_outputs(ctx, const_cast<uint32_t*>(d_ios), num_io, d_err));
            return SIPP_OK;
        }
        SIPP_TRY(sipp_mapg2_fill(ctx, a, d_ios, num_io, log_n, d_trace, d_err));
    } else if (a->kind == 6) {
        SIPP_TRY(sipp_pairing_fill(ctx, a, d_ios, num_io, log_n, d_trace, d_err));
        if (ctx->outputs_only) return SIPP_OK;
    } else if (a->kind == 2) {
        Fq12Cols c{1, 1 + 192, a->checked_base, cpl};
        col_bit = 1 + 384;
        col_e = col_bit + 1;
        exp_off = 192;
        ProfScope ps(ctx, "trace_fq12_chain");
        hipLaunchKernelGGL(fq12_chain_kernel, dim3(num_io), dim3(384), 0, ctx->stream, d_ios, num_io, d_trace, n, c);
        SIPP_CHECK_HIP(ctx, hipGetLastError());
    } else {
        const int ext = a->kind == 0 ? 1 : 2, ncl = 16 * ext;
        const int32_t* hard_lay = !a->hardened ? nullptr
                                  : a->kind == 0 ? (cpl == 1 ? AIR_HARD_LAYOUT_G1H_U16 : AIR_HARD_LAYOUT_G1H_U8)
                                                 : (cpl == 1 ? AIR_HARD_LAYOUT_G2H_U16 : AIR_HARD_LAYOUT_G2H_U8);
        const int hard_inf_col = hard_lay ? hard_lay[7] : 0;
        CurveCols c{1, 1 + ncl, 1 + 2 * ncl, 1 + 3 * ncl, a->checked_base, a->checked_base + ncl * cpl,
                    a->checked_base + 2 * ncl * cpl, cpl};
        col_bit = 1 + 4 * ncl;
        col_e = col_bit + 1;
        exp_off = 32 * ext;
        if (ext == 1) {
            RowPts<1>* rows = arena_alloc_t<RowPts<1>>(ctx, n);
            if (!rows) return SIPP_E_NOMEM;
            {
                ProfScope ps(ctx, "trace_curve_chain");
                hipLaunchKernelGGL((curve_dbl_par_kernel<1, 4>), dim3((num_io + 15) / 16), dim3(64), 0, ctx->stream, d_ios, num_io,
                                   (uint32_t)a->pi_per_io, rows);
                hipLaunchKernelGGL(curve_scan_kernel<1>, dim3(num_io), dim3(256), 0, ctx->stream, d_ios, num_io,
                                   (uint32_t)a->pi_per_io, rows);
            }
            SIPP_CHECK_HIP(ctx, hipGetLastError());
            gate_after_chain(ctx);
            if (ctx->outputs_only) {
                hipLaunchKernelGGL(curve_outputs_kernel<1>, dim3((num_io + 63) / 64), dim3(64), 0, ctx->stream, rows,
                                   const_cast<uint32_t*>(d_ios), num_io, (uint32_t)a->pi_per_io, d_err);
                SIPP_CHECK_HIP(ctx, hipGetLastError());
                return SIPP_OK;
            }
            ProfScope ps(ctx, "trace_curve_rows");
            hipLaunchKernelGGL(curve_rows_kernel<1>, dim3((unsigned)(n / ROWS_BLOCK)), dim3(ROWS_BLOCK), 0, ctx->stream, rows,
                               d_trace, n, c, a->hardened, hard_inf_col, d_err);
            SIPP_CHECK_HIP(ctx, hipGetLastError());
        } else {
            RowPts<2>* rows = arena_alloc_t<RowPts<2>>(ctx, n);
            if (!rows) return SIPP_E_NOMEM;
            {
                ProfScope ps(ctx, "trace_curve_chain");
                hipLaunchKernelGGL((curve_dbl_par_kernel<2, 8>), dim3((num_io + 7) / 8), dim3(64), 0, ctx->stream, d_ios, num_io,
                                   (uint32_t)a->pi_per_io, rows);
                hipLaunchKernelGGL(curve_scan_kernel<2>, dim3(num_io), dim3(256), 0, ctx->stream, d_ios, num_io,
                                   (uint32_t)a->pi_per_io, rows);
            }
            SIPP_CHECK_HIP(ctx, hipGetLastError());
            gate_after_chain(ctx);
            if (ctx->outputs_only) {
                hipLaunchKernelGGL(curve_outputs_kernel<2>, dim3((num_io + 63) / 64), dim3(64), 0, ctx->stream, rows,
                                   const_cast<uint32_t*>(d_ios), num_io, (uint32_t)a->pi_per_io, d_err);
                SIPP_CHECK_HIP(ctx, hipGetLastError());
                return SIPP_OK;
            }
            ProfScope ps(ctx, "trace_curve_rows");
            hipLaunchKernelGGL(curve_rows_kernel<2>, dim3((unsigned)(n / ROWS_BLOCK)), dim3(ROWS_BLOCK), 0, ctx->stream, rows,
                               d_trace, n, c, a->hardened, hard_inf_col, d_err);
            SIPP_CHECK_HIP(ctx, hipGetLastError());
// ... 154 lines not shown
```

Measured before the change: 2455 pairings/s.

## Use pinned chain staging, device-side power tables, and event-based cross-stream gating

Small device-to-host and host-to-device transfers (caps, openings, final poly, PoW result, error flag, query indices, gather tasks) now go through a pinned staging area instead of pageable stack or heap buffers. This avoids the staged copies the runtime makes for pageable memory. Alpha-power limb tables are built on the GPU by a new kernel instead of on the host, which removes one host loop and a synchronize. The gather-task upload is moved ahead of the PoW search. The cross-proof gate is released with a recorded HIP event before the stream synchronize, so the waiting stream can order on the event. Quotient segment metadata is cached per AIR, and aux coefficient staging uses pinned memory without an extra synchronize.

```diff
diff --git a/sipp_amd/csrc/api.hip b/sipp_amd/csrc/api.hip
--- a/sipp_amd/csrc/api.hip
+++ b/sipp_amd/csrc/api.hip
@@ -73,7 +73,14 @@
     if (hipMalloc((void**)&ctx->arena, workspace_bytes) != hipSuccess) return bail(SIPP_E_NOMEM);
     if (hipEventCreate(&ctx->t0) != hipSuccess || hipEventCreate(&ctx->t1) != hipSuccess) return bail(SIPP_E_HIP);
     ctx->h_pinned_words = (size_t)1 << 23;
-    if (hipHostMalloc((void**)&ctx->h_pinned, ctx->h_pinned_words * 8) != hipSuccess) return bail(SIPP_E_NOMEM);
+    if (hipHostMalloc((void**)&ctx->h_pinned, (ctx->h_pinned_words + SIPP_CHAIN_WORDS) * 8) != hipSuccess) return bail(SIPP_E_NOMEM);
+    ctx->h_chain = ctx->h_pinned + ctx->h_pinned_words;
+    for (hipEvent_t* e : {&ctx->ev_gate})
+        if (hipEventCreateWithFlags(e, hipEventDisableTiming) != hipSuccess) return bail(SIPP_E_HIP);
+    {
+        const char* e = getenv("SIPP_CHAIN_HOST_TABLES");
+        ctx->host_tables = e && atoi(e) != 0;
+    }
     int rc = sipp_poseidon_init_constants(ctx);
     if (rc != SIPP_OK) return bail(rc);
     *out = ctx;
@@ -98,6 +105,8 @@
     for (auto e : ctx->ev_pool) (void)hipEventDestroy(e);
     if (ctx->t0) (void)hipEventDestroy(ctx->t0);
     if (ctx->t1) (void)hipEventDestroy(ctx->t1);
+    for (hipEvent_t e : {ctx->ev_gate})
+        if (e) (void)hipEventDestroy(e);
     if (ctx->h_pinned) (void)hipHostFree(ctx->h_pinned);
     if (ctx->arena) (void)hipFree(ctx->arena);
     if (ctx->aux_stream) (void)hipStreamDestroy(ctx->aux_stream);
diff --git a/sipp_amd/csrc/ctx.hpp b/sipp_amd/csrc/ctx.hpp
--- a/sipp_amd/csrc/ctx.hpp
+++ b/sipp_amd/csrc/ctx.hpp
@@ -20,6 +20,7 @@
     std::mutex mu;
     std::condition_variable cv;
     bool open = false;
+    hipEvent_t ev = nullptr;
     void release() {
         {
             std::lock_guard<std::mutex> lk(mu);
@@ -33,6 +34,8 @@
     }
 };
 
+constexpr size_t SIPP_CHAIN_WORDS = (size_t)1 << 18, SIPP_CHAIN_POW = 1024, SIPP_CHAIN_ERR = 1025, SIPP_CHAIN_BUF = 2048;
+
 struct sipp_prof_entry {
     int calls = 0;
     double ms = 0.0;
@@ -50,6 +53,13 @@
     size_t arena_peak = 0;
 
     std::map<std::tuple<int, uint64_t, uint64_t>, uint64_t*> tables;
+
+    struct QuotientSegs {
+        int ns = 0, n_gadget_segs = 0;
+        std::vector<uint32_t> after;
+        const uint32_t* d_off = nullptr;
+    };
+    std::map<std::pair<uint64_t, uint64_t>, QuotientSegs> quotient_segs;
 
     bool prof = false;
     std::vector<hipEvent_t> ev_pool;
@@ -60,6 +70,9 @@
 
     uint64_t* h_pinned = nullptr;
     size_t h_pinned_words = 0;
+    uint64_t* h_chain = nullptr;
+    hipEvent_t ev_gate = nullptr;
+    bool host_tables = false;
 
     sipp_gate* gate_wait = nullptr;
     sipp_gate* gate_release = nullptr;
diff --git a/sipp_amd/csrc/fri.hip b/sipp_amd/csrc/fri.hip
--- a/sipp_amd/csrc/fri.hip
+++ b/sipp_amd/csrc/fri.hip
@@ -8,8 +8,9 @@
     const uint32_t ch = std::min(cap_height, log_leaves);
     uint64_t off = 0;
     for (uint32_t l = 0; l < log_leaves - ch; l++) off += (uint64_t)1 << (log_leaves - l);
-    SIPP_CHECK_HIP(ctx, hipMemcpyAsync(cap_host, d_tree + 4 * off, ((size_t)4 << ch) * 8, hipMemcpyDeviceToHost, ctx->stream));
+    SIPP_CHECK_HIP(ctx, hipMemcpyAsync(ctx->h_chain, d_tree + 4 * off, ((size_t)4 << ch) * 8, hipMemcpyDeviceToHost, ctx->stream));
     SIPP_CHECK_HIP(ctx, hipStreamSynchronize(ctx->stream));
+    memcpy(cap_host, ctx->h_chain, ((size_t)4 << ch) * 8);
     return SIPP_OK;
 }
 
@@ -75,8 +76,13 @@
     (void)cap_words;
     if (final_len) *final_len = len_c;
     {
-        std::vector<uint64_t> fpv(2 * len_c);
-        SIPP_CHECK_HIP(ctx, hipMemcpyAsync(fpv.data(), cur, fpv.size() * 8, hipMemcpyDeviceToHost, ctx->stream));
+        std::vector<uint64_t> big;
+        uint64_t* fpv = ctx->h_chain + SIPP_CHAIN_BUF;
+        if (2 * len_c > SIPP_CHAIN_WORDS - SIPP_CHAIN_BUF) {
+            big.resize(2 * len_c);
+            fpv = big.data();
+        }
+        SIPP_CHECK_HIP(ctx, hipMemcpyAsync(fpv, cur, 2 * len_c * 8, hipMemcpyDeviceToHost, ctx->stream));
         SIPP_CHECK_HIP(ctx, hipStreamSynchronize(ctx->stream));
         for (size_t i = 0; i < len_c; i++) {
             uint64_t e[2] = {fpv[i], fpv[len_c + i]};
@@ -85,23 +91,6 @@
         }
     }
     if (tick) tick("fri commit phase");
-    uint64_t pow_witness = 0;
-    if (p.pow_rule == SIPP_POW_HASH) {
-        uint64_t zero[12] = {0}, cur_h[4];
-        for (int i = 0; i < 4; i++) cur_h[i] = ch.get();
-        SIPP_TRY(sipp_k_pow_search(ctx, zero, cur_h, 4, 0, p.pow_bits, &pow_witness));
-    } else {
-        SIPP_TRY(sipp_k_pow_search(ctx, ch.state, ch.in_buf, ch.n_in, 7, p.pow_bits, &pow_witness));
-        ch.observe(pow_witness);
-        (void)ch.get();
-    }
-    SIPP_TRY(push(&pow_witness, 1));
-    if (tick) tick("pow");
-    std::vector<uint32_t> qidx(nq);
-    for (uint32_t i = 0; i < nq; i++) qidx[i] = (uint32_t)(ch.get() % m);
-    uint32_t* d_idx = arena_alloc_t<uint32_t>(ctx, nq);
-    if (!d_idx) return SIPP_E_NOMEM;
-    SIPP_CHECK_HIP(ctx, hipMemcpyAsync(d_idx, qidx.data(), nq * 4, hipMemcpyHostToDevice, ctx->stream));
     const uint32_t nsib0 = log_m - p.cap_height;
     size_t st_words = 0;
     std::vector<size_t> off_rows(n_oracles), off_sib(n_oracles), off_leaf(R), off_rsib(R);
@@ -129,22 +118,42 @@
     if (st_words > ctx->h_pinned_words) return sipp_fail(ctx, SIPP_E_NOMEM, "query staging exceeds the pinned buffer");
     uint64_t* d_st = arena_alloc_t<uint64_t>(ctx, st_words);
     if (!d_st) return SIPP_E_NOMEM;
-    std::vector<QueryGatherTask> tasks;
+    uint32_t* d_idx = arena_alloc_t<uint32_t>(ctx, nq);
+    if (!d_idx) return SIPP_E_NOMEM;
+    QueryGatherTask* d_tasks = nullptr;
+    uint32_t n_tasks = 0;
     {
+        QueryGatherTask* tasks = reinterpret_cast<QueryGatherTask*>(ctx->h_chain + SIPP_CHAIN_BUF + 512);
+        auto add = [&](const QueryGatherTask& t) { tasks[n_tasks++] = t; };
         for (int o = 0; o < n_oracles; o++) {
-            tasks.push_back(QueryGatherTask{ors[o].lde, d_st + off_rows[o], (uint64_t)ors[o].stride, 0, ors[o].ncols, 0, 0});
-            if (nsib0) tasks.push_back(QueryGatherTask{ors[o].tree, d_st + off_sib[o], 0, 1, log_m, nsib0, 0});
+            add(QueryGatherTask{ors[o].lde, d_st + off_rows[o], (uint64_t)ors[o].stride, 0, ors[o].ncols, 0, 0});
+            if (nsib0) add(QueryGatherTask{ors[o].tree, d_st + off_sib[o], 0, 1, log_m, nsib0, 0});
         }
         for (uint32_t r = 0; r < R; r++) {
             const uint32_t ab = p.arity_bits[r];
-            tasks.push_back(QueryGatherTask{r_vals[r], d_st + off_leaf[r], (uint64_t)1 << r_loglen[r], 2, rshift[r], ab, 0});
-            if (rsib[r]) tasks.push_back(QueryGatherTask{r_tree[r], d_st + off_rsib[r], 0, 1, r_loglen[r] - ab, rsib[r], rshift[r]});
-        }
-        QueryGatherTask* d_tasks = arena_alloc_t<QueryGatherTask>(ctx, tasks.size());
+            add(QueryGatherTask{r_vals[r], d_st + off_leaf[r], (uint64_t)1 << r_loglen[r], 2, rshift[r], ab, 0});
+            if (rsib[r]) add(QueryGatherTask{r_tree[r], d_st + off_rsib[r], 0, 1, r_loglen[r] - ab, rsib[r], rshift[r]});
+        }
+        d_tasks = arena_alloc_t<QueryGatherTask>(ctx, n_tasks);
         if (!d_tasks) return SIPP_E_NOMEM;
-        SIPP_CHECK_HIP(ctx, hipMemcpyAsync(d_tasks, tasks.data(), tasks.size() * sizeof(QueryGatherTask), hipMemcpyHostToDevice, ctx->stream));
-        SIPP_TRY(sipp_k_gather_tasks(ctx, d_tasks, (uint32_t)tasks.size(), d_idx, nq));
-    }
+        SIPP_CHECK_HIP(ctx, hipMemcpyAsync(d_tasks, tasks, n_tasks * sizeof(QueryGatherTask), hipMemcpyHostToDevice, ctx->stream));
+    }
+    uint64_t pow_witness = 0;
+    if (p.pow_rule == SIPP_POW_HASH) {
+        uint64_t zero[12] = {0}, cur_h[4];
+        for (int i = 0; i < 4; i++) cur_h[i] = ch.get();
+        SIPP_TRY(sipp_k_pow_search(ctx, zero, cur_h, 4, 0, p.pow_bits, &pow_witness));
+    } else {
+        SIPP_TRY(sipp_k_pow_search(ctx, ch.state, ch.in_buf, ch.n_in, 7, p.pow_bits, &pow_witness));
+        ch.observe(pow_witness);
+        (void)ch.get();
+    }
+    SIPP_TRY(push(&pow_witness, 1));
+    if (tick) tick("pow");
+    uint32_t* h_idx = reinterpret_cast<uint32_t*>(ctx->h_chain + SIPP_CHAIN_BUF);
+    for (uint32_t i = 0; i < nq; i++) h_idx[i] = (uint32_t)(ch.get() % m);
+    SIPP_CHECK_HIP(ctx, hipMemcpyAsync(d_idx, h_idx, nq * 4, hipMemcpyHostToDevice, ctx->stream));
+    SIPP_TRY(sipp_k_gather_tasks(ctx, d_tasks, n_tasks, d_idx, nq));
     uint64_t* hst = ctx->h_pinned;
     SIPP_CHECK_HIP(ctx, hipMemcpyAsync(hst, d_st, st_words * 8, hipMemcpyDeviceToHost, ctx->stream));
     SIPP_CHECK_HIP(ctx, hipStreamSynchronize(ctx->stream));
@@ -323,8 +332,13 @@
             SIPP_TRY(sipp_k_openings(ctx, oracles[rg.oracle].d_coeffs + (size_t)rg.col_begin * n, cnt, n, d_zp[b], nullptr, d_open + 4 * at));
             at += cnt;
         }
-        std::vector<uint64_t> hop(4 * k + 4);
-        SIPP_CHECK_HIP(ctx, hipMemcpyAsync(hop.data(), d_open, (4 * k) * 8, hipMemcpyDeviceToHost, ctx->stream));
+        std::vector<uint64_t> big;
+        uint64_t* hop = ctx->h_chain + SIPP_CHAIN_BUF;
+        if (4 * k > SIPP_CHAIN_WORDS - SIPP_CHAIN_BUF) {
+            big.resize(4 * k);
+            hop = big.data();
+        }
+        SIPP_CHECK_HIP(ctx, hipMemcpyAsync(hop, d_open, (4 * k) * 8, hipMemcpyDeviceToHost, ctx->stream));
         SIPP_CHECK_HIP(ctx, hipStreamSynchronize(ctx->stream));
         for (size_t j = 0; j < k; j++) {
             memcpy(pf + pos, &hop[4 * j], 16);
@@ -344,9 +358,9 @@
             const sipp_poly_range& rg = batches[b].ranges[r];
             for (uint32_t c = rg.col_begin; c < rg.col_end; c++) cols.push_back(oracles[rg.oracle].d_coeffs + (size_t)c * n);
         }
-        std::vector<uint32_t> apow(6 * k + 6);
-        gl::E2 ap = gl::e2(1);
-        for (size_t c = 0; c < k; c++) {
+        std::vector<uint32_t> apow(ctx->host_tables ? 6 * k + 6 : 0);
+        gl::E2 ap = ctx->host_tables ? gl::e2(1) : gl::pow(alpha, (uint64_t)k);
+        for (size_t c = 0; c < k && ctx->host_tables; c++) {
             const uint64_t comp[2] = {ap.c0, ap.c1};
             for (int q = 0; q < 2; q++) {
                 apow[6 * c + 3 * q] = (uint32_t)comp[q] & 0x3FFFFFu;
@@ -356,10 +370,13 @@
             ap = gl::mul(ap, alpha);
         }
         const uint64_t** d_cols = reinterpret_cast<const uint64_t**>(arena_alloc(ctx, (k + 1) * sizeof(uint64_t*)));
-        uint32_t* d_apow = arena_alloc_t<uint32_t>(ctx, apow.size());
+        uint32_t* d_apow = arena_alloc_t<uint32_t>(ctx, 6 * k + 6);
         if (!d_cols || !d_apow) return SIPP_E_NOMEM;
         SIPP_CHECK_HIP(ctx, hipMemcpyAsync(d_cols, cols.data(), k * sizeof(uint64_t*), hipMemcpyHostToDevice, ctx->stream));
-        SIPP_CHECK_HIP(ctx, hipMemcpyAsync(d_apow, apow.data(), apow.size() * 4, hipMemcpyHostToDevice, ctx->stream));
+        if (ctx->host_tables)
+            SIPP_CHECK_HIP(ctx, hipMemcpyAsync(d_apow, apow.data(), apow.size() * 4, hipMemcpyHostToDevice, ctx->stream));
+        else
+            SIPP_TRY(sipp_k_e2_pow_limbs(ctx, alpha, (int)k, d_apow));
         SIPP_CHECK_HIP(ctx, hipStreamSynchronize(ctx->stream));
         SIPP_TRY(sipp_k_fri_batch_quotient(ctx, d_cols, (int)k, n, d_apow, d_zp[b], d_zip[b], ap, b == 0, d_acc));
     }
diff --git a/sipp_amd/csrc/poseidon.hip b/sipp_amd/csrc/poseidon.hip
--- a/sipp_amd/csrc/poseidon.hip
+++ b/sipp_amd/csrc/poseidon.hip
@@ -296,7 +296,8 @@
     a.n_in = n_in; a.pow_bits = pow_bits; a.resp_word = resp_word; a.result = d_res;
     const uint32_t log_batch = pow_bits + 1 < 12 ? 12 : pow_bits + 1 > 28 ? 28 : pow_bits + 1;
     const uint64_t batch = (uint64_t)1 << log_batch;
-    unsigned long long h_res = ~0ull;
+    volatile unsigned long long& h_res = *reinterpret_cast<volatile unsigned long long*>(ctx->h_chain + SIPP_CHAIN_POW);
+    h_res = ~0ull;
     SIPP_CHECK_HIP(ctx, hipMemsetAsync(d_res, 0xff, sizeof(unsigned long long), ctx->stream));
     for (uint64_t base = 0; base < ((uint64_t)1 << 44); base += batch) {
         a.base = base;
@@ -305,7 +306,7 @@
             hipLaunchKernelGGL(pow_kernel, dim3((unsigned)(batch / 256)), dim3(256), 0, ctx->stream, a);
         }
         SIPP_CHECK_HIP(ctx, hipGetLastError());
-        SIPP_CHECK_HIP(ctx, hipMemcpyAsync(&h_res, d_res, sizeof h_res, hipMemcpyDeviceToHost, ctx->stream));
+        SIPP_CHECK_HIP(ctx, hipMemcpyAsync(ctx->h_chain + SIPP_CHAIN_POW, d_res, sizeof(unsigned long long), hipMemcpyDeviceToHost, ctx->stream));
         SIPP_CHECK_HIP(ctx, hipStreamSynchronize(ctx->stream));
         if (h_res != ~0ull) break;
     }
diff --git a/sipp_amd/csrc/prover.hip b/sipp_amd/csrc/prover.hip
--- a/sipp_amd/csrc/prover.hip
+++ b/sipp_amd/csrc/prover.hip
@@ -405,10 +405,22 @@
     a.part[((size_t)g * 2 + 1) * m + j] = gl::mul(c.acc1, a.seg_pow[2 * g + 1]);
 }
 
-__global__ void alpha_pow3_kernel(uint64_t a0, uint64_t a1, int K, int nc, uint32_t* __restrict__ out) {
+__global__ void alpha_pow3_kernel(uint64_t a0, uint64_t a1, int K, int nc, uint32_t* __restrict__ out, int ns,
+                                  const uint32_t* __restrict__ after, uint64_t* __restrict__ seg_pow, uint32_t* __restrict__ apoly3) {
     const int t = blockIdx.x * blockDim.x + threadIdx.x;
     const int total = 2 * 3 + nc * 2 * 6;
-    if (t >= total) return;
+    if (t >= total) {
+        const int u = t - total;
+        if (u < 2 * ns) {
+            seg_pow[u] = gl::pow(u & 1 ? a1 : a0, (uint64_t)after[u >> 1]);
+        } else if (u < 2 * ns + 128 && ns > 0) {
+            const int v = u - 2 * ns;
+            uint32_t l[3];
+            gl::limbs3(l, gl::pow(v >= 64 ? a1 : a0, (uint64_t)(v & 63)));
+            for (int q = 0; q < 3; q++) apoly3[3 * v + q] = l[q];
+        }
+        return;
+    }
     int c, e;
     if (t < 6) {
         c = t / 3;
@@ -767,6 +779,17 @@
         if (threadIdx.x < 4) a.partial[((size_t)(col_base + c0 + c) * gridDim.y + blockIdx.y) * 4 + threadIdx.x] = s[threadIdx.x][0];
         __syncthreads();
     }
+}
+
+__global__ void e2_pow_limbs_kernel(E2 a, int count, uint32_t* __restrict__ out) {
+    const int c = blockIdx.x * blockDim.x + threadIdx.x;
+    if (c >= count) return;
+    const E2 p = gl::pow(a, (uint64_t)c);
+    uint32_t l[3];
+    gl::limbs3(l, p.c0);
+    for (int q = 0; q < 3; q++) out[6 * c + q] = l[q];
+    gl::limbs3(l, p.c1);
+    for (int q = 0; q < 3; q++) out[6 * c + 3 + q] = l[q];
 }
 
 struct CombArgs {
@@ -1100,6 +1123,83 @@
     }
 }
 
+typedef sipp_ctx::QuotientSegs QuotientSegs;
+static int quotient_segments(sipp_ctx* ctx, const air_spec_t* a, const QuotientSegs** out) {
+    const auto key = std::make_pair((uint64_t)(a->kind + 8 * a->hardened), (uint64_t)a->table_bits);
+    auto it = ctx->quotient_segs.find(key);
+    if (it != ctx->quotient_segs.end()) {
+        *out = &it->second;
+        return SIPP_OK;
+    }
+    std::vector<uint32_t> off, cnt;
+    std::vector<int> ncons;
+    const int64_t* w = a->prog;
+    const int64_t* end = a->prog + a->prog_len;
+    while (w < end && w[0] == 1) {
+        off.push_back((uint32_t)(w - a->prog));
+        cnt.push_back(0);
+        if (w[6] != 2) return sipp_fail(ctx, SIPP_E_UNSUPPORTED, "quotient: gadgets must pair their limbs (group 2)");
+        ncons.push_back(32 / (int)w[6] + 1);
+        w += 7;
+        w += 2 + 5 * w[1];
+        int64_t np = *w++;
+        for (int64_t p = 0; p < np; p++) {
+            w += 1;
+            w += 2 + 5 * w[1];
+            w += 2 + 5 * w[1];
+        }
+        int64_t nl = *w++;
+        for (int64_t p = 0; p < nl; p++) {
+            w += 1;
+            w += 2 + 5 * w[1];
+        }
+        if (np > 64) {
+            const uint32_t nsl = (uint32_t)std::min<int64_t>(SIPP_QUOTIENT_MAX_SLICES, (np + 39) / 40);
+            cnt.back() = 0x80000000u | (nsl << 8);
+            for (uint32_t k = 1; k < nsl; k++) {
+                off.push_back(off.back());
+                cnt.push_back(0x80000000u | (nsl << 8) | k);
+                ncons.push_back(0);
+            }
+        }
+    }
+    while (w < end) {
+        off.push_back((uint32_t)(w - a->prog));
+        uint32_t k = 0;
+        while (w < end && k < 64) {
+            int64_t nmono = w[1];
+            w += 2;
+            for (int64_t mo = 0; mo < nmono; mo++) w += 2 + 2 * w[1];
+            k++;
+        }
+        cnt.push_back(k);
+        ncons.push_back((int)k);
+    }
+    QuotientSegs sg;
+    const int ns = (int)off.size();
+    sg.ns = ns;
+    auto is_gadget = [](uint32_t c) { return c == 0 || (c >> 31) != 0; };
+    while (sg.n_gadget_segs < ns && is_gadget(cnt[sg.n_gadget_segs])) sg.n_gadget_segs++;
+    for (int g = sg.n_gadget_segs; g < ns; g++)
+        if (is_gadget(cnt[g])) return sipp_fail(ctx, SIPP_E_UNSUPPORTED, "quotient: gadgets must precede the polynomial constraints");
+    sg.after.assign((size_t)ns, 0);
+    int after = 0;
+    for (int g = ns - 1; g >= 0; g--) {
+        sg.after[g] = (uint32_t)after;
+        after += ncons[g];
+    }
+    std::vector<uint64_t> packed(((size_t)3 * ns + 1) / 2 + 1, 0);
+    uint32_t* p32 = reinterpret_cast<uint32_t*>(packed.data());
+    memcpy(p32, off.data(), (size_t)ns * 4);
+    memcpy(p32 + ns, cnt.data(), (size_t)ns * 4);
+    memcpy(p32 + 2 * ns, sg.after.data(), (size_t)ns * 4);
+    uint64_t* t = nullptr;
+    SIPP_TRY(sipp_table_put(ctx, 108, key.first, key.second, packed, &t));
+    sg.d_off = reinterpret_cast<const uint32_t*>(t);
+    *out = &(ctx->quotient_segs[key] = std::move(sg));
+    return SIPP_OK;
+}
+
 int sipp_k_quotient(sipp_ctx* ctx, const air_spec_t* a, uint32_t log_n, const uint64_t* d_lde, const uint64_t* d_zlde,
                     size_t lde_stride, const uint64_t* d_aux, const uint64_t alpha[2], const uint64_t beta[2],
                     const uint64_t gamma[2], uint64_t* d_out) {
@@ -1192,100 +1292,46 @@
             x = gl::mul(x, gi);
         }
     }
-    int n_gadget_segs = 0;
+    const QuotientSegs* sg = nullptr;
+    SIPP_TRY(quotient_segments(ctx, a, &sg));
+    const int ns = sg->ns, n_gadget_segs = sg->n_gadget_segs;
+    q.n_seg = ns;
     ArenaScope scope(ctx);
-    {
-        std::vector<uint32_t> off, cnt;
-        std::vector<int> ncons;
-        const int64_t* w = a->prog;
-        const int64_t* end = a->prog + a->prog_len;
-        while (w < end && w[0] == 1) {
-            off.push_back((uint32_t)(w - a->prog));
-            cnt.push_back(0);
-            if (w[6] != 2) return sipp_fail(ctx, SIPP_E_UNSUPPORTED, "quotient: gadgets must pair their limbs (group 2)");
-            ncons.push_back(32 / (int)w[6] + 1);
-            w += 7;
-            w += 2 + 5 * w[1];
-            int64_t np = *w++;
-            for (int64_t p = 0; p < np; p++) {
-                w += 1;
-                w += 2 + 5 * w[1];
-                w += 2 + 5 * w[1];
+    uint64_t* d_tab = arena_alloc_t<uint64_t>(ctx, (size_t)2 * ns + 192);
+    q.part = arena_alloc_t<uint64_t>(ctx, (size_t)ns * 2 * m);
+    if (!d_tab || !q.part) return SIPP_E_NOMEM;
+    q.seg_pow = d_tab;
+    q.seg_off = sg->d_off;
+    q.seg_cnt = sg->d_off + ns;
+    q.apoly3 = reinterpret_cast<const uint32_t*>(d_tab + 2 * ns);
+    if (ctx->host_tables) {
+        uint64_t* host = ctx->h_chain + SIPP_CHAIN_BUF;
+        if ((size_t)2 * ns + 192 > SIPP_CHAIN_WORDS - SIPP_CHAIN_BUF) return sipp_fail(ctx, SIPP_E_NOMEM, "quotient: segment table exceeds the pinned staging");
+        for (int g = 0; g < ns; g++) {
+            host[2 * g] = gl::pow(alpha[0], (uint64_t)sg->after[g]);
+            host[2 * g + 1] = gl::pow(alpha[1], (uint64_t)sg->after[g]);
+        }
+        uint32_t* ap = reinterpret_cast<uint32_t*>(&host[2 * ns]);
+        for (int ch = 0; ch < 2; ch++) {
+            uint64_t x = 1;
+            for (int e = 0; e < 64; e++) {
+                ap[(ch * 64 + e) * 3 + 0] = (uint32_t)x & 0x3FFFFFu;
+                ap[(ch * 64 + e) * 3 + 1] = (uint32_t)(x >> 22) & 0x3FFFFFu;
+                ap[(ch * 64 + e) * 3 + 2] = (uint32_t)(x >> 44);
+                x = gl::mul(x, alpha[ch]);
             }
-            int64_t nl = *w++;
-            for (int64_t p = 0; p < nl; p++) {
-                w += 1;
-                w += 2 + 5 * w[1];
-            }
-            if (np > 64) {
-                const uint32_t nsl = (uint32_t)std::min<int64_t>(SIPP_QUOTIENT_MAX_SLICES, (np + 39) / 40);
-                cnt.back() = 0x80000000u | (nsl << 8);
-                for (uint32_t k = 1; k < nsl; k++) {
-                    off.push_back(off.back());
-                    cnt.push_back(0x80000000u | (nsl << 8) | k);
-                    ncons.push_back(0);
-                }
-            }
-        }
-        while (w < end) {
-            off.push_back((uint32_t)(w - a->prog));
-            uint32_t k = 0;
-            while (w < end && k < 64) {
-                int64_t nmono = w[1];
-                w += 2;
-                for (int64_t mo = 0; mo < nmono; mo++) w += 2 + 2 * w[1];
-                k++;
-            }
-            cnt.push_back(k);
-            ncons.push_back((int)k);
-        }
-        const int ns = (int)off.size();
-        q.n_seg = ns;
-        n_gadget_segs = 0;
-        auto is_gadget = [](uint32_t c) { return c == 0 || (c >> 31) != 0; };
-        while (n_gadget_segs < ns && is_gadget(cnt[n_gadget_segs])) n_gadget_segs++;
-        for (int g = n_gadget_segs; g < ns; g++)
-            if (is_gadget(cnt[g])) return sipp_fail(ctx, SIPP_E_UNSUPPORTED, "quotient: gadgets must precede the polynomial constraints");
-        std::vector<uint64_t> host((size_t)ns * 2 + ns + 2 + 192, 0);
-        int after = 0;
-        for (int g = ns - 1; g >= 0; g--) {
-            host[2 * g] = gl::pow(alpha[0], (uint64_t)after);
-            host[2 * g + 1] = gl::pow(alpha[1], (uint64_t)after);
-            after += ncons[g];
-        }
-        uint32_t* h32 = reinterpret_cast<uint32_t*>(&host[2 * ns]);
-        memcpy(h32, off.data(), (size_t)ns * 4);
-        memcpy(h32 + ns, cnt.data(), (size_t)ns * 4);
-        const size_t ap_at = (size_t)ns * 2 + (((size_t)2 * ns + 1) >> 1);
-        {
-            uint32_t* ap = reinterpret_cast<uint32_t*>(&host[ap_at]);
-            for (int ch = 0; ch < 2; ch++) {
-                uint64_t x = 1;
-                for (int e = 0; e < 64; e++) {
-                    ap[(ch * 64 + e) * 3 + 0] = (uint32_t)x & 0x3FFFFFu;
-                    ap[(ch * 64 + e) * 3 + 1] = (uint32_t)(x >> 22) & 0x3FFFFFu;
-                    ap[(ch * 64 + e) * 3 + 2] = (uint32_t)(x >> 44);
-                    x = gl::mul(x, alpha[ch]);
-                }
-            }
-        }
-        uint64_t* d_tab = arena_alloc_t<uint64_t>(ctx, host.size());
-        q.part = arena_alloc_t<uint64_t>(ctx, (size_t)ns * 2 * m);
-        if (!d_tab || !q.part) return SIPP_E_NOMEM;
-        SIPP_CHECK_HIP(ctx, hipMemcpyAsync(d_tab, host.data(), host.size() * 8, hipMemcpyHostToDevice, ctx->stream));
+        }
+        SIPP_CHECK_HIP(ctx, hipMemcpyAsync(d_tab, host, ((size_t)2 * ns + 192) * 8, hipMemcpyHostToDevice, ctx->stream));
         SIPP_CHECK_HIP(ctx, hipStreamSynchronize(ctx->stream));
-        q.seg_pow = d_tab;
-        q.seg_off = reinterpret_cast<const uint32_t*>(d_tab + 2 * ns);
-        q.seg_cnt = q.seg_off + ns;
-        q.apoly3 = reinterpret_cast<const uint32_t*>(d_tab + ap_at);
     }
     {
         q.K = 3 + 6 * a->n_checked;
         const int nw = 6 + 12 * a->n_checked;
         uint32_t* d_ap = arena_alloc_t<uint32_t>(ctx, (size_t)3 * nw);
         if (!d_ap) return SIPP_E_NOMEM;
-        hipLaunchKernelGGL(alpha_pow3_kernel, dim3((unsigned)((nw + 255) / 256)), dim3(256), 0, ctx->stream, alpha[0], alpha[1],
-                           q.K, a->n_checked, d_ap);
+        const int ns_k = ctx->host_tables ? 0 : ns, lanes = nw + (ns_k ? 2 * ns_k + 128 : 0);
+        hipLaunchKernelGGL(alpha_pow3_kernel, dim3((unsigned)((lanes + 255) / 256)), dim3(256), 0, ctx->stream, alpha[0], alpha[1],
+                           q.K, a->n_checked, d_ap, ns_k, sg->d_off + 2 * ns, d_tab, reinterpret_cast<uint32_t*>(d_tab + 2 * ns));
         q.apow3 = d_ap;
         q.alphaK[0] = gl::pow(alpha[0], (uint64_t)q.K);
         q.alphaK[1] = gl::pow(alpha[1], (uint64_t)q.K);
@@ -1389,6 +1435,13 @@
     hipLaunchKernelGGL(openings_group_kernel, dim3(groups, (unsigned)segs), dim3(256), 0, ctx->stream, g);
     hipLaunchKernelGGL(openings_fold_kernel, dim3((4 * total + 255) / 256), dim3(256), 0, ctx->stream, g.partial, (uint32_t)total,
                        (uint32_t)segs, d_out);
+    SIPP_CHECK_HIP(ctx, hipGetLastError());
+    return SIPP_OK;
+}
+
+int sipp_k_e2_pow_limbs(sipp_ctx* ctx, gl::E2 a, int count, uint32_t* d_out) {
+    if (count <= 0) return SIPP_OK;
+    hipLaunchKernelGGL(e2_pow_limbs_kernel, dim3((unsigned)((count + 255) / 256)), dim3(256), 0, ctx->stream, a, count, d_out);
     SIPP_CHECK_HIP(ctx, hipGetLastError());
     return SIPP_OK;
 }
diff --git a/sipp_amd/csrc/prover.hpp b/sipp_amd/csrc/prover.hpp
--- a/sipp_amd/csrc/prover.hpp
+++ b/sipp_amd/csrc/prover.hpp
@@ -24,6 +24,7 @@
 constexpr int SIPP_QUOTIENT_MAX_SLICES = 8;
 int sipp_k_openings3(sipp_ctx* ctx, const uint64_t* const d_coeffs[3], const uint32_t ncols[3], size_t n, const uint64_t* d_t0,
                      const uint64_t* d_t1, uint64_t* d_out);
+int sipp_k_e2_pow_limbs(sipp_ctx* ctx, gl::E2 a, int count, uint32_t* d_out);
 int sipp_k_fri_final(sipp_ctx* ctx, const uint64_t* const src[3], const int cnt[3], size_t n, const uint32_t* d_apow3,
                      int n1, gl::E2 shift1, const uint64_t* d_zp[2], const uint64_t* d_zip[2], uint64_t* d_final);
 int sipp_k_fri_batch_quotient(sipp_ctx* ctx, const uint64_t* const* d_cols, int total, size_t n, const uint32_t* d_apow3,
diff --git a/sipp_amd/csrc/stark.hip b/sipp_amd/csrc/stark.hip
--- a/sipp_amd/csrc/stark.hip
+++ b/sipp_amd/csrc/stark.hip
@@ -85,8 +85,9 @@
     const uint32_t ch = std::min(ctx->cfg.cap_height, log_leaves);
     uint64_t off = 0;
     for (uint32_t l = 0; l < log_leaves - ch; l++) off += (uint64_t)1 << (log_leaves - l);
-    SIPP_CHECK_HIP(ctx, hipMemcpyAsync(cap_host, d_tree + 4 * off, ((size_t)4 << ch) * 8, hipMemcpyDeviceToHost, ctx->stream));
+    SIPP_CHECK_HIP(ctx, hipMemcpyAsync(ctx->h_chain, d_tree + 4 * off, ((size_t)4 << ch) * 8, hipMemcpyDeviceToHost, ctx->stream));
     SIPP_CHECK_HIP(ctx, hipStreamSynchronize(ctx->stream));
+    memcpy(cap_host, ctx->h_chain, ((size_t)4 << ch) * 8);
     return SIPP_OK;
 }
 
@@ -312,6 +313,9 @@
               arena_alloc_t<uint64_t>(ctx, tree_words(log_m)), P};
     Oracle3 Qo{arena_alloc_t<uint64_t>(ctx, (size_t)2 * mq), arena_alloc_t<uint64_t>(ctx, (size_t)Q * m),
                arena_alloc_t<uint64_t>(ctx, tree_words(log_m)), Q};
+    const int n_aux = a->n_aux;
+    const size_t nio = s.num_io;
+    if ((size_t)n_aux * nio > ctx->h_pinned_words) return sipp_fail(ctx, SIPP_E_NOMEM, "public-input polynomials larger than the pinned staging buffer");
     if (!d_err || !d_trace || !T.coeffs || !T.lde || !T.tree || !Z.coeffs || !Z.lde || !Z.tree || !Qo.coeffs || !Qo.lde ||
         !Qo.tree)
         return SIPP_E_NOMEM;
@@ -320,19 +324,22 @@
     SIPP_CHECK_HIP(ctx, hipMemsetAsync(d_err, 0, sizeof(int), ctx->stream));
     SIPP_TRY(sipp_trace_fill(ctx, a, d_ios, s.num_io, log_n, d_trace, d_err));
     {
-        int h_err = 0;
-        SIPP_CHECK_HIP(ctx, hipMemcpyAsync(&h_err, d_err, sizeof(int), hipMemcpyDeviceToHost, ctx->stream));
+        volatile int* h_err = reinterpret_cast<volatile int*>(ctx->h_chain + SIPP_CHAIN_ERR);
+        SIPP_CHECK_HIP(ctx, hipMemcpyAsync(const_cast<int*>(h_err), d_err, sizeof(int), hipMemcpyDeviceToHost, ctx->stream));
+        if (ctx->gate_release) {
+            SIPP_CHECK_HIP(ctx, hipEventRecord(ctx->ev_gate, ctx->stream));
+            ctx->gate_release->ev = ctx->ev_gate;
+            ctx->gate_release->release();
+            ctx->gate_release = nullptr;
+        }
         SIPP_CHECK_HIP(ctx, hipStreamSynchronize(ctx->stream));
-        if (h_err) return sipp_fail(ctx, h_err, "trace fill: IO record not provable (claimed output wrong, degenerate point or non-canonical limbs)");
+        if (*h_err) return sipp_fail(ctx, *h_err, "trace fill: IO record not provable (claimed output wrong, degenerate point or non-canonical limbs)");
     }
 
     tick("trace fill");
-    if (ctx->gate_release) {
-        ctx->gate_release->release();
-        ctx->gate_release = nullptr;
-    }
     if (ctx->gate_wait) {
         ctx->gate_wait->wait();
+        if (ctx->gate_wait->ev) SIPP_CHECK_HIP(ctx, hipStreamWaitEvent(ctx->stream, ctx->gate_wait->ev, 0));
         ctx->gate_wait = nullptr;
     }
     uint64_t cap_host[4 << 8];
@@ -348,10 +355,9 @@
         pi_root(pis.data(), s.num_io, a->pi_per_io, root);
         ch.observe_many(root, 4);
     }
-    const int n_aux = a->n_aux;
     const uint32_t log_io = log_n - (uint32_t)a->log_rows;
-    const size_t nio = s.num_io;
-    std::vector<uint64_t> auxc((size_t)n_aux * nio), col(nio);
+    uint64_t* auxc = ctx->h_pinned;
+    std::vector<uint64_t> col(nio);
     {
         const uint64_t g = gl::root_of_unity(log_n);
         for (int ai = 0; ai < n_aux; ai++) {
@@ -411,9 +417,8 @@
         uint64_t* d_auxc = arena_alloc_t<uint64_t>(ctx, (size_t)n_aux * nio + 1);
         uint64_t* d_aux = arena_alloc_t<uint64_t>(ctx, (size_t)n_aux * mq + 1);
         if (!d_auxc || !d_aux) return SIPP_E_NOMEM;
-        SIPP_CHECK_HIP(ctx, hipMemcpyAsync(d_auxc, auxc.data(), auxc.size() * 8, hipMemcpyHostToDevice, ctx->stream));
-        SIPP_CHECK_HIP(ctx, hipStreamSynchronize(ctx->stream));
         if (n_aux) {
+            SIPP_CHECK_HIP(ctx, hipMemcpyAsync(d_auxc, auxc, (size_t)n_aux * nio * 8, hipMemcpyHostToDevice, ctx->stream));
             int rc_aux = sipp_tree_coset_eval(ctx, d_auxc, d_aux, (size_t)n_aux, log_io, log_mq);
             if (rc_aux == SIPP_E_UNSUPPORTED)
                 rc_aux = sipp_ntt_dif(ctx, d_auxc, nio, log_io, d_aux, mq, log_mq, (size_t)n_aux, false, NttDiag{gl::GEN, 0});
@@ -441,14 +446,14 @@
         SIPP_TRY(sipp_k_pow_table4(ctx, bases, n, tabs));
     }
     {
+        const size_t cols = (size_t)(W + P + Q);
+        if (cols * 4 > SIPP_CHAIN_WORDS - SIPP_CHAIN_BUF) return sipp_fail(ctx, SIPP_E_NOMEM, "opening set larger than the pinned staging");
         const uint64_t* const cf[3] = {T.coeffs, Z.coeffs, Qo.coeffs};
         const uint32_t nc3[3] = {(uint32_t)W, (uint32_t)P, (uint32_t)Q};
         SIPP_TRY(sipp_k_openings3(ctx, cf, nc3, n, d_zp[0], d_zp[1], d_open));
-    }
-    std::vector<uint64_t> hop((size_t)(W + P + Q) * 4);
-    SIPP_CHECK_HIP(ctx, hipMemcpyAsync(hop.data(), d_open, hop.size() * 8, hipMemcpyDeviceToHost, ctx->stream));
-    SIPP_CHECK_HIP(ctx, hipStreamSynchronize(ctx->stream));
-    {
+        const uint64_t* hop = ctx->h_chain + SIPP_CHAIN_BUF;
+        SIPP_CHECK_HIP(ctx, hipMemcpyAsync(ctx->h_chain + SIPP_CHAIN_BUF, d_open, cols * 32, hipMemcpyDeviceToHost, ctx->stream));
+        SIPP_CHECK_HIP(ctx, hipStreamSynchronize(ctx->stream));
         for (int c = 0; c < W; c++) push(&hop[(size_t)c * 4], 2);
         for (int c = 0; c < W; c++) push(&hop[(size_t)c * 4 + 2], 2);
         for (int c = 0; c < P; c++) push(&hop[(size_t)(W + c) * 4], 2);
@@ -465,21 +470,26 @@
     const gl::E2 fa = ch.get_ext();
     uint64_t* d_final = arena_alloc_t<uint64_t>(ctx, 2 * n);
     {
-        std::vector<uint32_t> apow((size_t)(W + P + Q) * 6);
-        gl::E2 ap = gl::e2(1);
-        for (int c = 0; c < W + P + Q; c++) {
-            const uint64_t comp[2] = {ap.c0, ap.c1};
-            for (int q = 0; q < 2; q++) {
-                apow[6 * c + 3 * q] = (uint32_t)comp[q] & 0x3FFFFFu;
-                apow[6 * c + 3 * q + 1] = (uint32_t)(comp[q] >> 22) & 0x3FFFFFu;
-                apow[6 * c + 3 * q + 2] = (uint32_t)(comp[q] >> 44);
+        const int total = W + P + Q;
+        uint32_t* d_apow = arena_alloc_t<uint32_t>(ctx, (size_t)total * 6);
+        if (!d_final || !d_apow) return SIPP_E_NOMEM;
+        if (!ctx->host_tables) {
+            SIPP_TRY(sipp_k_e2_pow_limbs(ctx, fa, total, d_apow));
+        } else {
+            uint32_t* apow = reinterpret_cast<uint32_t*>(ctx->h_chain + SIPP_CHAIN_BUF);
+            gl::E2 ap = gl::e2(1);
+            for (int c = 0; c < total; c++) {
+                const uint64_t comp[2] = {ap.c0, ap.c1};
+                for (int q = 0; q < 2; q++) {
+                    apow[6 * c + 3 * q] = (uint32_t)comp[q] & 0x3FFFFFu;
+                    apow[6 * c + 3 * q + 1] = (uint32_t)(comp[q] >> 22) & 0x3FFFFFu;
+                    apow[6 * c + 3 * q + 2] = (uint32_t)(comp[q] >> 44);
+                }
+                ap = gl::mul(ap, fa);
             }
-            ap = gl::mul(ap, fa);
-        }
-        uint32_t* d_apow = arena_alloc_t<uint32_t>(ctx, apow.size());
-        if (!d_final || !d_apow) return SIPP_E_NOMEM;
-        SIPP_CHECK_HIP(ctx, hipMemcpyAsync(d_apow, apow.data(), apow.size() * 4, hipMemcpyHostToDevice, ctx->stream));
-        SIPP_CHECK_HIP(ctx, hipStreamSynchronize(ctx->stream));
+            SIPP_CHECK_HIP(ctx, hipMemcpyAsync(d_apow, apow, (size_t)total * 24, hipMemcpyHostToDevice, ctx->stream));
+            SIPP_CHECK_HIP(ctx, hipStreamSynchronize(ctx->stream));
+        }
         const uint64_t* src[3] = {T.coeffs, Z.coeffs, Qo.coeffs};
         const int cnt[3] = {W, P, Q};
         const uint64_t* zp[2] = {d_zp[0], d_zp[1]};
diff --git a/sipp_amd/csrc/trace.hip b/sipp_amd/csrc/trace.hip
--- a/sipp_amd/csrc/trace.hip
+++ b/sipp_amd/csrc/trace.hip
@@ -1208,6 +1208,7 @@
 static void gate_after_chain(sipp_ctx* ctx) {
     if (ctx->gate_wait) {
         ctx->gate_wait->wait();
+        if (ctx->gate_wait->ev) (void)hipStreamWaitEvent(ctx->stream, ctx->gate_wait->ev, 0);
         ctx->gate_wait = nullptr;
     }
 }
```

Result: no change. 2457 pairings/s (median of 3 runs) (+0.1%).
